# argmaxinc/WhisperKit

Hardware: AMD Instinct MI355X
Metric: audio-sec/sec (1/RTF), 30 s chunks: host PCM -> log-mel + encoder + greedy decode -> segments (higher is better)
Workload: dtype f16

## Files before the change

whisperkit_amd/csrc/epi_stage.h:

```cpp
#pragma once

#if defined(__HIPCC__)
#define WH_EPI_FN __host__ __device__ inline __attribute__((always_inline))
#else
#define WH_EPI_FN inline
#endif

namespace wh {
namespace epi {

constexpr int kWaveRegion = 16384;

constexpr int kRow16 = 144;
WH_EPI_FN int f16_write_off(int lane, int i2, int j, int g) { return (i2 * 32 + (lane & 31)) * kRow16 + j * 64 + g * 16 + (lane >> 5) * 8; }
WH_EPI_FN int f16_read_row(int lane, int it) { return it * 8 + (lane >> 3); }
WH_EPI_FN int f16_read_col(int lane) { return (lane & 7) * 8; }
WH_EPI_FN int f16_read_off(int lane, int it) { return f16_read_row(lane, it) * kRow16 + f16_read_col(lane) * 2; }

constexpr int kRow32 = 272;
WH_EPI_FN int f32_write_off(int lane, int j, int g) { return (lane & 31) * kRow32 + j * 128 + g * 32 + (lane >> 5) * 16; }
WH_EPI_FN int f32_read_row(int lane, int it) { return it * 4 + (lane >> 4); }
WH_EPI_FN int f32_read_col(int lane) { return (lane & 15) * 4; }
WH_EPI_FN int f32_read_off(int lane, int it) { return f32_read_row(lane, it) * kRow32 + f32_read_col(lane) * 4; }

constexpr int kRowT = 272;
WH_EPI_FN int vt_write_off(int lane, int i, int g) { return (lane & 31) * kRowT + (i * 32 + g * 8 + (lane >> 5) * 4) * 2; }
WH_EPI_FN int vt_read_col(int lane, int it) { return it * 4 + (lane >> 4); }
WH_EPI_FN int vt_read_row(int lane) { return (lane & 15) * 8; }
WH_EPI_FN int vt_read_off(int lane, int it) { return vt_read_col(lane, it) * kRowT + vt_read_row(lane) * 2; }

static_assert(64 * kRow16 <= kWaveRegion && 32 * kRow32 <= kWaveRegion && 32 * kRowT <= kWaveRegion, "a pass fits the wave's slice");

constexpr int kSplitStage = 3 * 16384;
WH_EPI_FN int split_swz(int row) { return (row >> 2) & 3; }
WH_EPI_FN int split_dma_row(int tid) { return tid >> 2; }
WH_EPI_FN int split_dma_chunk(int tid) { return (tid & 3) ^ split_swz(split_dma_row(tid)); }
WH_EPI_FN int split_read_off(int row, int chunk) { return row * 64 + ((chunk ^ split_swz(row)) * 16); }
static_assert(2 * kSplitStage <= 8 * kWaveRegion, "the split stages fit the launch's 128 KB (the staged epilogues' slices)");

}
}
```

whisperkit_amd/csrc/gemm.hip:

```cpp
#include <algorithm>
#include <cstdlib>
#include <type_traits>

#include "epi_stage.h"
#include "kernels.h"
#include "knobs.h"

namespace wh {

constexpr int BK = 32;
constexpr int LDT = 40;

template <int EPI, int TM, int TN, bool SPLIT = false>
__device__ __forceinline__ void gemm_epilogue(const GemmArgs& a, f32x16 (&acc)[TM][TN], int m_wave, int n_wave, int lane) {
#pragma unroll
    for (int j = 0; j < TN; ++j) {
        const int n = n_wave + j * 32 + (lane & 31);
        if (n >= a.N) continue;
        const float bias = a.bias ? a.bias[n] : 0.0f;
#pragma unroll
        for (int i = 0; i < TM; ++i) {
            const int mb = m_wave + i * 32 + 4 * (lane >> 5);
#pragma unroll
            for (int g = 0; g < 4; ++g) {
                const int mg = mb + 8 * g;
                if (mg >= a.M) continue;
                float v[4];
#pragma unroll
                for (int r = 0; r < 4; ++r) v[r] = acc[i][j][g * 4 + r] + bias;
                if constexpr (EPI == EPI_QKV_ENC) {
                    const int d = a.d_model;
                    if (n >= 2 * d) {
                        int call = n - 2 * d;
                        int bb = mg / kCtx, t = mg - bb * kCtx;
                        if (t + 3 < kCtx) {
                            f16x4 pk = {(f16)v[0], (f16)v[1], (f16)v[2], (f16)v[3]};
                            *reinterpret_cast<f16x4*>(a.vt16 + ((size_t)bb * d + call) * kCtxPad + t) = pk;
                        } else {
                            for (int r = 0; r < 4; ++r) {
                                int m = mg + r;
                                if (m < a.M) { int b2 = m / kCtx, t2 = m - b2 * kCtx; a.vt16[((size_t)b2 * d + call) * kCtxPad + t2] = (f16)v[r]; }
                            }
                        }
                        continue;
                    }
                }
#pragma unroll
                for (int r = 0; r < 4; ++r) {
                    const int m = mg + r;
                    if (m >= a.M) continue;
                    const float x = v[r];
                    if constexpr (EPI == EPI_F16) {
                        a.out16[(size_t)m * a.ldc + n] = (f16)x;
                    } else if constexpr (EPI == EPI_GELU_F16) {
                        if constexpr (SPLIT) { f16 h_, l_; split_f16(gelu_erf_fast(x), h_, l_); a.out16[(size_t)m * a.ldc + n] = h_; a.out16_lo[(size_t)m * a.ldc + n] = l_; }
                        else a.out16[(size_t)m * a.ldc + n] = (f16)gelu_erf_fast(x);
                    } else if constexpr (EPI == EPI_RESID_F32) {
                        a.out32[(size_t)m * a.ldc + n] += x;
                    } else if constexpr (EPI == EPI_F32) {
                        a.out32[(size_t)m * a.ldc + n] = x;
                    } else if constexpr (EPI == EPI_QKV_ENC) {
                        const int d = a.d_model;
                        if (n < d) a.out16[(size_t)m * d + n] = (f16)x;
                        else a.k16[(size_t)m * d + (n - d)] = (f16)x;
                    } else if constexpr (EPI == EPI_CROSS_KV) {
                        const int d = a.d_model, H = d >> 6;
                        const int l = n / (2 * d), rem = n - l * 2 * d, kv = rem >= d, hc = rem - kv * d;
                        const int bb = m / kCtx, t = m - bb * kCtx;
                        const size_t o = ((((size_t)l * a.max_batch + bb) * H + (hc >> 6)) * kCtx + t) * kHeadDim + (hc & 63);
                        f16 hi_; signed char lo_;
                        hr24_encode(x, hi_, lo_);
                        (kv ? a.kv_v_hi : a.kv_k_hi)[o] = hi_;
                        (kv ? a.kv_v_lo : a.kv_k_lo)[o] = lo_;
                    } else if constexpr (EPI == EPI_CONV1) {
                        int bb = m / a.rows_per_batch_out, t = m - bb * a.rows_per_batch_out;
                        if constexpr (SPLIT) {
                            const size_t o = ((size_t)bb * kFramesPad + t + 1) * a.ldc + n;
                            f16 h_, l_; split_f16(gelu_erf_fast(x), h_, l_); a.out16[o] = h_; a.out16_lo[o] = l_;
                        } else {
                            a.out16[((size_t)bb * kFramesPad + t + 1) * a.ldc + n] = (f16)gelu_erf_fast(x);
                        }
                    } else if constexpr (EPI == EPI_CONV2) {
                        int t = m % a.rows_per_batch_out;
                        a.out32[(size_t)m * a.ldc + n] = gelu_erf_fast(x) + a.pos[(size_t)t * a.ldc + n];
                    }
                }
            }
        }
    }
}

__device__ __forceinline__ void load_tile_bias(const GemmArgs& a, float4 (&bias)[2][4], int nw, int lane) {
#pragma unroll
    for (int j = 0; j < 2; ++j)
#pragma unroll
        for (int g = 0; g < 4; ++g) bias[j][g] = float4{0, 0, 0, 0};
    if (a.bias) {
#pragma unroll
        for (int j = 0; j < 2; ++j)
#pragma unroll
            for (int g = 0; g < 4; ++g) bias[j][g] = *reinterpret_cast<const float4*>(a.bias + nw + j * 32 + 8 * g + 4 * (lane >> 5));
    }
}

__device__ __forceinline__ void split_f16x4(float v0, float v1, float v2, float v3, f16x4& hi, f16x4& lo) {
    f16 h_, l_;
    split_f16(v0, h_, l_); hi[0] = h_; lo[0] = l_;
    split_f16(v1, h_, l_); hi[1] = h_; lo[1] = l_;
    split_f16(v2, h_, l_); hi[2] = h_; lo[2] = l_;
    split_f16(v3, h_, l_); hi[3] = h_; lo[3] = l_;
}

template <int EPI, int TM, int TN, bool BATCH_BIAS = false, bool SPLIT = false>
__device__ __forceinline__ void gemm_epilogue_swapped(const GemmArgs& a, f32x16 (&acc)[TM][TN], int m_wave, int n_wave, int lane) {
    float4 tile_bias[2][4];
    if constexpr (BATCH_BIAS) {
        static_assert(TM == 4 && TN == 2, "wave tile of gemm256_kernel");
        if (n_wave >= a.N) return;
        load_tile_bias(a, tile_bias, n_wave, lane);
    }
#pragma unroll
    for (int i = 0; i < TM; ++i) {
        const int m = m_wave + i * 32 + (lane & 31);
        if (m >= a.M) continue;
        int bb = 0, t = m;
        if constexpr (EPI == EPI_CROSS_KV) { bb = m / kCtx; t = m - bb * kCtx; }
        if constexpr (EPI == EPI_CONV1 || EPI == EPI_CONV2) { bb = m / a.rows_per_batch_out; t = m - bb * a.rows_per_batch_out; }
#pragma unroll
        for (int j = 0; j < TN; ++j) {
#pragma unroll
            for (int g = 0; g < 4; ++g) {
                const int n = n_wave + j * 32 + 8 * g + 4 * (lane >> 5);
                if (n >= a.N) continue;
                float4 bias = float4{0, 0, 0, 0};
                if constexpr (BATCH_BIAS) bias = tile_bias[j][g];
                else if (a.bias) bias = *reinterpret_cast<const float4*>(a.bias + n);
                float v0 = acc[i][j][4 * g] + bias.x, v1 = acc[i][j][4 * g + 1] + bias.y;
                float v2 = acc[i][j][4 * g + 2] + bias.z, v3 = acc[i][j][4 * g + 3] + bias.w;
                if constexpr (EPI == EPI_F16) {
                    *reinterpret_cast<f16x4*>(a.out16 + (size_t)m * a.ldc + n) = f16x4{(f16)v0, (f16)v1, (f16)v2, (f16)v3};
                } else if constexpr (EPI == EPI_GELU_F16) {
                    if constexpr (SPLIT) {
                        f16x4 hi, lo;
                        split_f16x4(gelu_erf_fast(v0), gelu_erf_fast(v1), gelu_erf_fast(v2), gelu_erf_fast(v3), hi, lo);
                        *reinterpret_cast<f16x4*>(a.out16 + (size_t)m * a.ldc + n) = hi;
                        *reinterpret_cast<f16x4*>(a.out16_lo + (size_t)m * a.ldc + n) = lo;
                    } else {
                        *reinterpret_cast<f16x4*>(a.out16 + (size_t)m * a.ldc + n) =
                            f16x4{(f16)gelu_erf_fast(v0), (f16)gelu_erf_fast(v1), (f16)gelu_erf_fast(v2), (f16)gelu_erf_fast(v3)};
                    }
                } else if constexpr (EPI == EPI_RESID_F32) {
                    float4* p = reinterpret_cast<float4*>(a.out32 + (size_t)m * a.ldc + n);
                    float4 o = *p;
                    o.x += v0; o.y += v1; o.z += v2; o.w += v3;
                    *p = o;
                } else if constexpr (EPI == EPI_F32) {
                    *reinterpret_cast<float4*>(a.out32 + (size_t)m * a.ldc + n) = float4{v0, v1, v2, v3};
                } else if constexpr (EPI == EPI_QKV_ENC) {
                    const int d = a.d_model;
                    f16* dst = n < d ? a.out16 + (size_t)m * d + n : a.k16 + (size_t)m * d + (n - d);
                    *reinterpret_cast<f16x4*>(dst) = f16x4{(f16)v0, (f16)v1, (f16)v2, (f16)v3};
                } else if constexpr (EPI == EPI_CROSS_KV) {
                    const int d = a.d_model, H = d >> 6;
                    const int l = n / (2 * d), rem = n - l * 2 * d, kv = rem >= d, hc = rem - kv * d;
                    const size_t o = ((((size_t)l * a.max_batch + bb) * H + (hc >> 6)) * kCtx + t) * kHeadDim + (hc & 63);
                    f16x4 hi4; char4 lo4;
                    { f16 h_; signed char l_; hr24_encode(v0, h_, l_); hi4[0] = h_; lo4.x = l_; hr24_encode(v1, h_, l_); hi4[1] = h_; lo4.y = l_;
                      hr24_encode(v2, h_, l_); hi4[2] = h_; lo4.z = l_; hr24_encode(v3, h_, l_); hi4[3] = h_; lo4.w = l_; }
                    *reinterpret_cast<f16x4*>((kv ? a.kv_v_hi : a.kv_k_hi) + o) = hi4;
                    *reinterpret_cast<char4*>((kv ? a.kv_v_lo : a.kv_k_lo) + o) = lo4;
                } else if constexpr (EPI == EPI_CONV1) {
                    if constexpr (SPLIT) {
                        const size_t o = ((size_t)bb * kFramesPad + t + 1) * a.ldc + n;
                        f16x4 hi, lo;
                        split_f16x4(gelu_erf_fast(v0), gelu_erf_fast(v1), gelu_erf_fast(v2), gelu_erf_fast(v3), hi, lo);
                        *reinterpret_cast<f16x4*>(a.out16 + o) = hi;
                        *reinterpret_cast<f16x4*>(a.out16_lo + o) = lo;
                    } else {
                        *reinterpret_cast<f16x4*>(a.out16 + ((size_t)bb * kFramesPad + t + 1) * a.ldc + n) =
                            f16x4{(f16)gelu_erf_fast(v0), (f16)gelu_erf_fast(v1), (f16)gelu_erf_fast(v2), (f16)gelu_erf_fast(v3)};
                    }
                } else if constexpr (EPI == EPI_CONV2) {
                    const float4 ps = *reinterpret_cast<const float4*>(a.pos + (size_t)t * a.ldc + n);
                    *reinterpret_cast<float4*>(a.out32 + (size_t)m * a.ldc + n) =
                        float4{gelu_erf_fast(v0) + ps.x, gelu_erf_fast(v1) + ps.y, gelu_erf_fast(v2) + ps.z, gelu_erf_fast(v3) + ps.w};
                }
            }
        }
    }
}

template <int BM, int BN, int EPI, bool SPLIT>
__device__ __forceinline__ void gemm_main(const GemmArgs& a) {
    constexpr int WM = BM / 2, WN = BN / 2, TM = WM / 32, TN = WN / 32;
    constexpr int CA = BM * 4 / 256, CB = BN * 4 / 256;
    __shared__ __attribute__((aligned(16))) f16 As[SPLIT ? 4 : 2][BM * LDT];
    __shared__ __attribute__((aligned(16))) f16 Bs[2][BN * LDT];

    const int tid = threadIdx.x, lane = tid & 63, wave = tid >> 6;
    const int wm = wave >> 1, wn = wave & 1;
    const int m0 = blockIdx.y * BM, n0 = blockIdx.x * BN;

    const f16* a_ptr[CA];
    const f16* a_lo_ptr[SPLIT ? CA : 1];
    bool a_ok[CA];
    int a_lds[CA];
#pragma unroll
    for (int i = 0; i < CA; ++i) {
        int c = tid + 256 * i, row = c >> 2, cc = c & 3;
        int m = m0 + row;
        a_ok[i] = m < a.M;
        int mm = a_ok[i] ? m : 0;
        long long off = (long long)(mm / a.a_rows_per_batch) * a.a_batch_stride + (long long)(mm % a.a_rows_per_batch) * a.lda;
        a_ptr[i] = a.A + off + cc * 8;
        if constexpr (SPLIT) a_lo_ptr[i] = a.A_lo + off + cc * 8;
        a_lds[i] = row * LDT + cc * 8;
    }
    const f16* b_ptr[CB];
    bool b_ok[CB];
    int b_lds[CB];
#pragma unroll
    for (int i = 0; i < CB; ++i) {
        int c = tid + 256 * i, row = c >> 2, cc = c & 3;
        int n = n0 + row;
        b_ok[i] = n < a.N;
        b_ptr[i] = a.W + (long long)(b_ok[i] ? n : 0) * a.K + cc * 8;
        b_lds[i] = row * LDT + cc * 8;
    }
    const int kc = (tid & 3) * 8;

    uint4 ra[CA], rb[CB], ral[SPLIT ? CA : 1];
    auto gload = [&](int k0) {
        bool kin = (k0 + kc) < a.K;
#pragma unroll
        for (int i = 0; i < CA; ++i) ra[i] = (a_ok[i] && kin) ? *reinterpret_cast<const uint4*>(a_ptr[i] + k0) : uint4{0, 0, 0, 0};
        if constexpr (SPLIT) {
#pragma unroll
            for (int i = 0; i < CA; ++i) ral[i] = (a_ok[i] && kin) ? *reinterpret_cast<const uint4*>(a_lo_ptr[i] + k0) : uint4{0, 0, 0, 0};
        }
#pragma unroll
        for (int i = 0; i < CB; ++i) rb[i] = (b_ok[i] && kin) ? *reinterpret_cast<const uint4*>(b_ptr[i] + k0) : uint4{0, 0, 0, 0};
    };
    auto lstore = [&](int buf) {
#pragma unroll
        for (int i = 0; i < CA; ++i) *reinterpret_cast<uint4*>(&As[buf][a_lds[i]]) = ra[i];
#pragma unroll
        for (int i = 0; i < CB; ++i) *reinterpret_cast<uint4*>(&Bs[buf][b_lds[i]]) = rb[i];
        if constexpr (SPLIT) {
#pragma unroll
            for (int i = 0; i < CA; ++i) *reinterpret_cast<uint4*>(&As[2 + buf][a_lds[i]]) = ral[i];
        }
    };

    const int nk = (a.K + BK - 1) / BK;
    const int fr = lane & 31, fk = (lane >> 5) * 8;
    auto body = [&](auto swap_tag) {
        constexpr bool SWAP = decltype(swap_tag)::value;
        f32x16 acc[TM][TN];
#pragma unroll
        for (int i = 0; i < TM; ++i)
#pragma unroll
            for (int j = 0; j < TN; ++j)
#pragma unroll
                for (int r = 0; r < 16; ++r) acc[i][j][r] = 0.0f;
        gload(0);
        lstore(0);
        __syncthreads();
        for (int kt = 0; kt < nk; ++kt) {
            const int cur = kt & 1;
            if (kt + 1 < nk) gload((kt + 1) * BK);
#pragma unroll
            for (int ks = 0; ks < 2; ++ks) {
                f16x8 af[TM], bf[TN];
#pragma unroll
                for (int i = 0; i < TM; ++i) af[i] = *reinterpret_cast<const f16x8*>(&As[cur][(wm * WM + i * 32 + fr) * LDT + ks * 16 + fk]);
#pragma unroll
                for (int j = 0; j < TN; ++j) bf[j] = *reinterpret_cast<const f16x8*>(&Bs[cur][(wn * WN + j * 32 + fr) * LDT + ks * 16 + fk]);
                f16x8 afl[SPLIT ? TM : 1];
                if constexpr (SPLIT) {
#pragma unroll
                    for (int i = 0; i < TM; ++i) afl[i] = *reinterpret_cast<const f16x8*>(&As[2 + cur][(wm * WM + i * 32 + fr) * LDT + ks * 16 + fk]);
                }
#pragma unroll
                for (int i = 0; i < TM; ++i)
#pragma unroll
                    for (int j = 0; j < TN; ++j) {
                        if constexpr (SWAP) acc[i][j] = __builtin_amdgcn_mfma_f32_32x32x16_f16(bf[j], af[i], acc[i][j], 0, 0, 0);
                        else acc[i][j] = __builtin_amdgcn_mfma_f32_32x32x16_f16(af[i], bf[j], acc[i][j], 0, 0, 0);
                        if constexpr (SPLIT) {
                            if constexpr (SWAP) acc[i][j] = __builtin_amdgcn_mfma_f32_32x32x16_f16(bf[j], afl[i], acc[i][j], 0, 0, 0);
                            else acc[i][j] = __builtin_amdgcn_mfma_f32_32x32x16_f16(afl[i], bf[j], acc[i][j], 0, 0, 0);
                        }
                    }
            }
            if (kt + 1 < nk) lstore(cur ^ 1);
            __syncthreads();
        }
        if constexpr (SWAP) gemm_epilogue_swapped<EPI, TM, TN, false, SPLIT>(a, acc, m0 + wm * WM, n0 + wn * WN, lane);
        else gemm_epilogue<EPI, TM, TN, SPLIT>(a, acc, m0 + wm * WM, n0 + wn * WN, lane);
    };
    if constexpr (EPI == EPI_QKV_ENC) {
        if (n0 + wn * WN >= 2 * a.d_model) body(std::false_type{});
        else body(std::true_type{});
    } else {
        body(std::true_type{});
    }
}

template <int BM, int BN, int EPI>
__global__ __launch_bounds__(256, 2) void gemm_kernel(const GemmArgs a) { gemm_main<BM, BN, EPI, false>(a); }
template <int BM, int BN, int EPI>
__global__ __launch_bounds__(256, 2) void gemm_split_kernel(const GemmArgs a) { gemm_main<BM, BN, EPI, true>(a); }

__device__ __forceinline__ void wave_lds_turn() {
    __builtin_amdgcn_fence(__ATOMIC_RELEASE, "wavefront");
    __builtin_amdgcn_wave_barrier();
    __builtin_amdgcn_fence(__ATOMIC_ACQUIRE, "wavefront");
}

template <int EPI, bool SPLIT = false>
__device__ __forceinline__ void epi_staged_f16(const GemmArgs& a, f32x16 (&acc)[4][2], unsigned char* wl, int mw, int nw, int lane) {
    if (nw >= a.N) return;
    f16* base = a.out16;
    int ld = a.ldc, nc = nw;
    if constexpr (EPI == EPI_QKV_ENC) {
        ld = a.d_model;
        if (nw >= ld) { base = a.k16; nc = nw - ld; }
    }
    float4 bias[2][4];
    load_tile_bias(a, bias, nw, lane);
    static_assert(!SPLIT || EPI == EPI_GELU_F16, "split output planes: GELU(fc1) only");
#pragma unroll
    for (int hh = 0; hh < 2; ++hh) {
#pragma unroll
        for (int plane = 0; plane < (SPLIT ? 2 : 1); ++plane) {
#pragma unroll
            for (int i2 = 0; i2 < 2; ++i2)
#pragma unroll
                for (int j = 0; j < 2; ++j)
#pragma unroll
                    for (int g = 0; g < 4; ++g) {
                        const f32x16& c = acc[2 * hh + i2][j];
                        const float v0 = c[4 * g] + bias[j][g].x, v1 = c[4 * g + 1] + bias[j][g].y, v2 = c[4 * g + 2] + bias[j][g].z, v3 = c[4 * g + 3] + bias[j][g].w;
                        f16x4 pk;
                        if constexpr (SPLIT) {
                            f16x4 hi, lo;
                            split_f16x4(gelu_erf_fast(v0), gelu_erf_fast(v1), gelu_erf_fast(v2), gelu_erf_fast(v3), hi, lo);
                            pk = plane ? lo : hi;
                        } else if constexpr (EPI == EPI_GELU_F16) pk = f16x4{(f16)gelu_erf_fast(v0), (f16)gelu_erf_fast(v1), (f16)gelu_erf_fast(v2), (f16)gelu_erf_fast(v3)};
                        else pk = f16x4{(f16)v0, (f16)v1, (f16)v2, (f16)v3};
                        *reinterpret_cast<f16x4*>(wl + epi::f16_write_off(lane, i2, j, g)) = pk;
                    }
            wave_lds_turn();
            f16* const dst = SPLIT && plane ? a.out16_lo : base;
#pragma unroll
            for (int it = 0; it < 8; ++it) {
                const int m = mw + hh * 64 + epi::f16_read_row(lane, it);
                const uint4 v = *reinterpret_cast<const uint4*>(wl + epi::f16_read_off(lane, it));
                if (m < a.M) *reinterpret_cast<uint4*>(dst + (size_t)m * ld + nc + epi::f16_read_col(lane)) = v;
            }
            wave_lds_turn();
        }
    }
}

__device__ __forceinline__ void epi_staged_resid(const GemmArgs& a, f32x16 (&acc)[4][2], unsigned char* wl, int mw, int nw, int lane) {
    if (nw >= a.N) return;
    float4 bias[2][4];
    load_tile_bias(a, bias, nw, lane);
#pragma unroll
    for (int i = 0; i < 4; ++i) {
        const int m_first = mw + i * 32 + epi::f32_read_row(lane, 0);
        float* const col0 = a.out32 + nw + epi::f32_read_col(lane);
        float4 old[8];
#pragma unroll
        for (int it = 0; it < 8; ++it) old[it] = *reinterpret_cast<const float4*>(col0 + (size_t)min(m_first + it * 4, a.M - 1) * a.ldc);
#pragma unroll
        for (int j = 0; j < 2; ++j)
#pragma unroll
            for (int g = 0; g < 4; ++g) {
                const f32x16& c = acc[i][j];
                *reinterpret_cast<float4*>(wl + epi::f32_write_off(lane, j, g)) =
                    float4{c[4 * g] + bias[j][g].x, c[4 * g + 1] + bias[j][g].y, c[4 * g + 2] + bias[j][g].z, c[4 * g + 3] + bias[j][g].w};
            }
        wave_lds_turn();
#pragma unroll
        for (int it = 0; it < 8; ++it) {
            const float4 v = *reinterpret_cast<const float4*>(wl + epi::f32_read_off(lane, it));
            float4 o = old[it];
            o.x += v.x; o.y += v.y; o.z += v.z; o.w += v.w;
            if (m_first + it * 4 < a.M) *reinterpret_cast<float4*>(col0 + (size_t)(m_first + it * 4) * a.ldc) = o;
        }
        wave_lds_turn();
    }
}

__device__ __forceinline__ void epi_staged_vt(const GemmArgs& a, f32x16 (&acc)[4][2], unsigned char* wl, int mw, int nw, int lane) {
    if (nw >= a.N) return;
    const int d = a.d_model;
    float bias2[2] = {0.0f, 0.0f};
    if (a.bias) { bias2[0] = a.bias[nw + (lane & 31)]; bias2[1] = a.bias[nw + 32 + (lane & 31)]; }
#pragma unroll
    for (int j = 0; j < 2; ++j) {
        const float bias = bias2[j];
#pragma unroll
        for (int i = 0; i < 4; ++i)
#pragma unroll
            for (int g = 0; g < 4; ++g) {
                const f32x16& c = acc[i][j];
                *reinterpret_cast<f16x4*>(wl + epi::vt_write_off(lane, i, g)) =
                    f16x4{(f16)(c[4 * g] + bias), (f16)(c[4 * g + 1] + bias), (f16)(c[4 * g + 2] + bias), (f16)(c[4 * g + 3] + bias)};
            }
        wave_lds_turn();
#pragma unroll
        for (int it = 0; it < 8; ++it) {
            const uint4 v = *reinterpret_cast<const uint4*>(wl + epi::vt_read_off(lane, it));
            const int call = nw - 2 * d + j * 32 + epi::vt_read_col(lane, it);
            const int m = mw + epi::vt_read_row(lane);
            if (m < a.M) {
                const int bb = m / kCtx, t = m - bb * kCtx;
                *reinterpret_cast<uint2*>(a.vt16 + ((size_t)bb * d + call) * kCtxPad + t) = uint2{v.x, v.y};
            }
            if (m + 4 < a.M) {
                const int bb = (m + 4) / kCtx, t = m + 4 - bb * kCtx;
                *reinterpret_cast<uint2*>(a.vt16 + ((size_t)bb * d + call) * kCtxPad + t) = uint2{v.z, v.w};
            }
        }
        wave_lds_turn();
    }
}

template <int EPI>
constexpr bool kHasStagedEpilogue = plan::has_staged_epilogue(EPI);

template <int EPI, int MODE, bool SPLIT>
__device__ __forceinline__ void gemm256_main(const GemmArgs& a) {
    constexpr int TM = 4, TN = 2;
    constexpr int STAGE = SPLIT ? epi::kSplitStage : 65536;
    constexpr int NP = SPLIT ? 6 : 8;
    extern __shared__ __attribute__((aligned(1024))) unsigned char smem[];
    const int tid = threadIdx.x, lane = tid & 63, wave = tid >> 6;
    const int wm = wave >> 2, wn = wave & 3;

    const int nwg = gridDim.x, orig = blockIdx.x;
    const int xcd = orig & 7, q = nwg >> 3, r = nwg & 7;
    const int wg = (xcd < r ? xcd * (q + 1) : r * (q + 1) + (xcd - r) * q) + (orig >> 3);
    const int tiles_n = (a.N + 255) >> 8, tiles_m = (a.M + 255) >> 8;
    constexpr int GM = 8;
    const int gsz = GM * tiles_n, grp = wg / gsz, first_m = grp * GM;
    const int gm = min(tiles_m - first_m, GM), in_g = wg - grp * gsz;
    const int m0 = (first_m + in_g % gm) << 8, n0 = (in_g / gm) << 8;

    const f16* src[NP];
    if constexpr (SPLIT) {
        const int srow = epi::split_dma_row(tid);
        const int chunk = epi::split_dma_chunk(tid);
#pragma unroll
        for (int j = 0; j < 2; ++j) {
            const int m = min(m0 + j * 128 + srow, a.M - 1);
            const long long off = (long long)(m / a.a_rows_per_batch) * a.a_batch_stride + (long long)(m % a.a_rows_per_batch) * a.lda + chunk * 8;
            src[j] = a.A + off;
            src[2 + j] = a.A_lo + off;
            const int n = min(n0 + j * 128 + srow, a.N - 1);
            src[4 + j] = a.W + (long long)n * a.K + chunk * 8;
        }
    } else {
        const int srow = tid >> 3;
        const int chunk = (tid & 7) ^ ((tid >> 4) & 7);
#pragma unroll
        for (int j = 0; j < 4; ++j) {
            const int m = min(m0 + j * 64 + srow, a.M - 1);
            src[j] = a.A + (long long)(m / a.a_rows_per_batch) * a.a_batch_stride + (long long)(m % a.a_rows_per_batch) * a.lda + chunk * 8;
            const int n = min(n0 + j * 64 + srow, a.N - 1);
            src[4 + j] = a.W + (long long)n * a.K + chunk * 8;
        }
    }
    auto piece = [&](int p, int kt) {
        if constexpr (SPLIT) {
            unsigned char* dst = smem + (kt & 1) * STAGE + wave * 1024 + (p >> 1) * 16384 + (p & 1) * 8192;
            __builtin_amdgcn_global_load_lds((const __attribute__((address_space(1))) void*)(src[p] + kt * 32),
                                             (__attribute__((address_space(3))) void*)dst, 16, 0, 0);
        } else {
            unsigned char* dst = smem + (kt & 1) * 65536 + wave * 1024 + (p >> 2) * 32768 + (p & 3) * 8192;
            __builtin_amdgcn_global_load_lds((const __attribute__((address_space(1))) void*)(src[p] + kt * 64),
                                             (__attribute__((address_space(3))) void*)dst, 16, 0, 0);
        }
    };

    const int fr = lane & 31, fh = lane >> 5, swz = SPLIT ? epi::split_swz(fr) : (fr >> 1) & 7;
    const int a_row_off = SPLIT ? (wm * 128 + fr) * 64 : (wm * 128 + fr) * 128, b_row_off = SPLIT ? 32768 + (wn * 64 + fr) * 64 : 32768 + (wn * 64 + fr) * 128;
    const int nk = SPLIT ? a.K >> 5 : a.K >> 6;
#define PP_BAR() do { __builtin_amdgcn_sched_barrier(0); asm volatile("s_barrier" ::: "memory"); __builtin_amdgcn_sched_barrier(0); } while (0)
#define PP_XBAR() do { __builtin_amdgcn_sched_barrier(0); asm volatile("s_waitcnt lgkmcnt(0)\n\ts_barrier" ::: "memory"); __builtin_amdgcn_sched_barrier(0); } while (0)
#define PP_VMWAIT() do { __builtin_amdgcn_sched_barrier(0); asm volatile("s_waitcnt vmcnt(0)" ::: "memory"); } while (0)
    auto body = [&](auto swap_tag) {
        constexpr bool SWAP = decltype(swap_tag)::value;
        f32x16 acc[TM][TN];
#pragma unroll
        for (int i = 0; i < TM; ++i)
#pragma unroll
            for (int j = 0; j < TN; ++j)
#pragma unroll
                for (int e = 0; e < 16; ++e) acc[i][j][e] = 0.0f;
        f16x8 af[2][TM], bf[2][TN];
        auto X = [&](int kt, int h) {
            if constexpr (SPLIT) {
                const unsigned char* sb = smem + (kt & 1) * STAGE;
                const int slot = ((2 * h + fh) ^ swz) * 16;
#pragma unroll
                for (int j = 0; j < TN; ++j) bf[0][j] = *reinterpret_cast<const f16x8*>(sb + b_row_off + j * 2048 + slot);
#pragma unroll
                for (int i = 0; i < TM; ++i) af[0][i] = *reinterpret_cast<const f16x8*>(sb + a_row_off + i * 2048 + slot);
#pragma unroll
                for (int i = 0; i < TM; ++i) af[1][i] = *reinterpret_cast<const f16x8*>(sb + 16384 + a_row_off + i * 2048 + slot);
            } else {
                const unsigned char* sb = smem + (kt & 1) * 65536;
#pragma unroll
                for (int s2 = 0; s2 < 2; ++s2) {
                    const int slot = ((2 * (2 * h + s2) + fh) ^ swz) * 16;
#pragma unroll
                    for (int j = 0; j < TN; ++j) bf[s2][j] = *reinterpret_cast<const f16x8*>(sb + b_row_off + j * 4096 + slot);
#pragma unroll
                    for (int i = 0; i < TM; ++i) af[s2][i] = *reinterpret_cast<const f16x8*>(sb + a_row_off + i * 4096 + slot);
                }
            }
        };
        auto Y = [&](auto dma_tag, int dma_kt) {
            constexpr bool DMA = decltype(dma_tag)::value;
            __builtin_amdgcn_s_setprio(1);
            if constexpr (SPLIT) {
#pragma unroll
                for (int i = 0; i < TM; ++i) {
#pragma unroll
                    for (int j = 0; j < TN; ++j) {
#pragma unroll
                        for (int pl = 0; pl < 2; ++pl) {
                            if constexpr (SWAP) acc[i][j] = __builtin_amdgcn_mfma_f32_32x32x16_f16(bf[0][j], af[pl][i], acc[i][j], 0, 0, 0);
                            else acc[i][j] = __builtin_amdgcn_mfma_f32_32x32x16_f16(af[pl][i], bf[0][j], acc[i][j], 0, 0, 0);
                        }
                    }
                    if constexpr (DMA) {
                        __builtin_amdgcn_sched_barrier(0);
                        if (i < 2) { piece(2 * i, dma_kt); piece(2 * i + 1, dma_kt); }
                        else piece(2 + i, dma_kt);
                        __builtin_amdgcn_sched_barrier(0);
                    }
                }
            } else {
#pragma unroll
                for (int s2 = 0; s2 < 2; ++s2)
#pragma unroll
                    for (int i = 0; i < TM; ++i) {
#pragma unroll
                        for (int j = 0; j < TN; ++j) {
                            if constexpr (SWAP) acc[i][j] = __builtin_amdgcn_mfma_f32_32x32x16_f16(bf[s2][j], af[s2][i], acc[i][j], 0, 0, 0);
                            else acc[i][j] = __builtin_amdgcn_mfma_f32_32x32x16_f16(af[s2][i], bf[s2][j], acc[i][j], 0, 0, 0);
                        }
                        if constexpr (DMA) { __builtin_amdgcn_sched_barrier(0); piece(s2 * 4 + i, dma_kt); __builtin_amdgcn_sched_barrier(0); }
                    }
            }
            __builtin_amdgcn_s_setprio(0);
        };
        constexpr std::true_type kDma{};
        constexpr std::false_type kNoDma{};
#pragma unroll
        for (int p = 0; p < NP; ++p) piece(p, 0);
        PP_VMWAIT();
        PP_BAR();
        if (wm == 0) {
            for (int t = 0; t + 1 < nk; ++t) {
                X(t, 0); PP_XBAR();
                Y(kDma, t + 1); PP_BAR();
                X(t, 1); PP_XBAR();
                Y(kNoDma, 0); PP_VMWAIT(); PP_BAR();
            }
            X(nk - 1, 0); PP_XBAR();
            Y(kNoDma, 0); PP_BAR();
            X(nk - 1, 1); PP_XBAR();
            Y(kNoDma, 0); PP_BAR();
            PP_BAR();
        } else {
            if (nk > 1) {
#pragma unroll
                for (int p = 0; p < NP; ++p) piece(p, 1);
            }
            PP_BAR();
            for (int t = 0; t + 2 < nk; ++t) {
                X(t, 0); PP_XBAR();
                Y(kNoDma, 0); PP_BAR();
                X(t, 1); PP_VMWAIT(); PP_XBAR();
                Y(kDma, t + 2); PP_BAR();
            }
            for (int t = max(nk - 2, 0); t < nk; ++t) {
                X(t, 0); PP_XBAR();
                Y(kNoDma, 0); PP_BAR();
                X(t, 1); PP_VMWAIT(); PP_XBAR();
                Y(kNoDma, 0); PP_BAR();
            }
        }
        if constexpr (MODE == 1 && kHasStagedEpilogue<EPI>) {
            unsigned char* wl = smem + wave * epi::kWaveRegion;
            if constexpr (!SWAP) epi_staged_vt(a, acc, wl, m0 + wm * 128, n0 + wn * 64, lane);
            else if constexpr (EPI == EPI_RESID_F32) epi_staged_resid(a, acc, wl, m0 + wm * 128, n0 + wn * 64, lane);
            else epi_staged_f16<EPI, SPLIT && EPI == EPI_GELU_F16>(a, acc, wl, m0 + wm * 128, n0 + wn * 64, lane);
        } else if constexpr (SWAP) gemm_epilogue_swapped<EPI, TM, TN, MODE == 2, SPLIT>(a, acc, m0 + wm * 128, n0 + wn * 64, lane);
        else gemm_epilogue<EPI, TM, TN, SPLIT>(a, acc, m0 + wm * 128, n0 + wn * 64, lane);
    };
#undef PP_BAR
#undef PP_XBAR
#undef PP_VMWAIT
    if constexpr (EPI == EPI_QKV_ENC) {
        if (n0 + wn * 64 >= 2 * a.d_model) body(std::false_type{});
        else body(std::true_type{});
    } else {
        body(std::true_type{});
    }
}

template <int EPI, int MODE>
__global__ __launch_bounds__(512) void gemm256_kernel(const GemmArgs a) { gemm256_main<EPI, MODE, false>(a); }
template <int EPI, int MODE>
__global__ __launch_bounds__(512) void gemm256_split_kernel(const GemmArgs a) { gemm256_main<EPI, MODE, true>(a); }


constexpr int kPersistWaveRegion = 12288;
static_assert(64 * epi::kRow16 <= kPersistWaveRegion && 32 * epi::kRow32 <= kPersistWaveRegion && 32 * epi::kRowT <= kPersistWaveRegion, "a pass fits the wave's slice");
template <int EPI, int MODE>
__global__ __launch_bounds__(512) void gemm256p_kernel(const GemmArgs a, int n_tiles, int stagger, int GM) {
    constexpr int TM = 4, TN = 2;
    extern __shared__ __attribute__((aligned(1024))) unsigned char smem[];
    const int tid = threadIdx.x, lane = tid & 63, wave = tid >> 6;
    const int wm = wave >> 2, wn = wave & 3;

    const int orig = blockIdx.x, xcd = orig & 7, q = n_tiles >> 3, r = n_tiles & 7;
    const int lo = xcd < r ? xcd * (q + 1) : r * (q + 1) + (xcd - r) * q, cnt = q + (xcd < r ? 1 : 0);
    const int per_xcd = gridDim.x >> 3;
    int it = orig >> 3;
    if (it >= cnt) return;
    if (stagger > 0) {
        const int rank = (it & 7) * 4 + ((it >> 3) & 3);
        for (int i = 0; i < rank * stagger; ++i) __builtin_amdgcn_s_sleep(1);
    }
    const int tiles_n = (a.N + 255) >> 8, tiles_m = (a.M + 255) >> 8;
    int m0, n0;
    auto tile_origin = [&](int wg, int& m0_, int& n0_) {
        const int gsz = GM * tiles_n, grp = wg / gsz, first_m = grp * GM;
        const int gm = min(tiles_m - first_m, GM), in_g = wg - grp * gsz;
        m0_ = (first_m + in_g % gm) << 8; n0_ = (in_g / gm) << 8;
    };
    const int srow = tid >> 3;
    const int chunk = (tid & 7) ^ ((tid >> 4) & 7);
    const f16* src[8];
    auto set_src = [&](int m0_, int n0_) {
#pragma unroll
        for (int j = 0; j < 4; ++j) {
            const int m = min(m0_ + j * 64 + srow, a.M - 1);
            src[j] = a.A + (long long)(m / a.a_rows_per_batch) * a.a_batch_stride + (long long)(m % a.a_rows_per_batch) * a.lda + chunk * 8;
            const int n = min(n0_ + j * 64 + srow, a.N - 1);
            src[4 + j] = a.W + (long long)n * a.K + chunk * 8;
        }
    };
    tile_origin(lo + it, m0, n0);
    set_src(m0, n0);
    auto piece = [&](int p, int kt) {
        unsigned char* dst = smem + (kt & 1) * 65536 + wave * 1024 + (p >> 2) * 32768 + (p & 3) * 8192;
        __builtin_amdgcn_global_load_lds((const __attribute__((address_space(1))) void*)(src[p] + kt * 64),
                                         (__attribute__((address_space(3))) void*)dst, 16, 0, 0);
    };

    const int fr = lane & 31, fh = lane >> 5, swz = (fr >> 1) & 7;
    const int a_row_off = (wm * 128 + fr) * 128, b_row_off = 32768 + (wn * 64 + fr) * 128;
    const int nk = a.K >> 6;
#define PP_BAR() do { __builtin_amdgcn_sched_barrier(0); asm volatile("s_barrier" ::: "memory"); __builtin_amdgcn_sched_barrier(0); } while (0)
#define PP_XBAR() do { __builtin_amdgcn_sched_barrier(0); asm volatile("s_waitcnt lgkmcnt(0)\n\ts_barrier" ::: "memory"); __builtin_amdgcn_sched_barrier(0); } while (0)
#define PP_VMWAIT() do { __builtin_amdgcn_sched_barrier(0); if (stagger != -2) asm volatile("s_waitcnt vmcnt(0)" ::: "memory"); } while (0)
    bool have_next = false;
    int m0n = 0, n0n = 0;
    auto body = [&](auto swap_tag) {
        constexpr bool SWAP = decltype(swap_tag)::value;
        f32x16 acc[TM][TN];
#pragma unroll
        for (int i = 0; i < TM; ++i)
#pragma unroll
            for (int j = 0; j < TN; ++j)
#pragma unroll
                for (int e = 0; e < 16; ++e) acc[i][j][e] = 0.0f;
        f16x8 af[2][TM], bf[2][TN];
        auto X = [&](int kt, int h) {
            const unsigned char* sb = smem + (kt & 1) * 65536;
#pragma unroll
            for (int s2 = 0; s2 < 2; ++s2) {
                const int slot = ((2 * (2 * h + s2) + fh) ^ swz) * 16;
#pragma unroll
                for (int j = 0; j < TN; ++j) bf[s2][j] = *reinterpret_cast<const f16x8*>(sb + b_row_off + j * 4096 + slot);
#pragma unroll
                for (int i = 0; i < TM; ++i) af[s2][i] = *reinterpret_cast<const f16x8*>(sb + a_row_off + i * 4096 + slot);
            }
        };
        auto Y = [&](auto dma_tag, int dma_kt) {
            constexpr bool DMA = decltype(dma_tag)::value;
            __builtin_amdgcn_s_setprio(1);
#pragma unroll
            for (int s2 = 0; s2 < 2; ++s2)
#pragma unroll
                for (int i = 0; i < TM; ++i) {
#pragma unroll
                    for (int j = 0; j < TN; ++j) {
                        if constexpr (SWAP) acc[i][j] = __builtin_amdgcn_mfma_f32_32x32x16_f16(bf[s2][j], af[s2][i], acc[i][j], 0, 0, 0);
                        else acc[i][j] = __builtin_amdgcn_mfma_f32_32x32x16_f16(af[s2][i], bf[s2][j], acc[i][j], 0, 0, 0);
                    }
                    if constexpr (DMA) { __builtin_amdgcn_sched_barrier(0); if (stagger != -1) piece(s2 * 4 + i, dma_kt); __builtin_amdgcn_sched_barrier(0); }
                }
            __builtin_amdgcn_s_setprio(0);
        };
        constexpr std::true_type kDma{};
        constexpr std::false_type kNoDma{};
        PP_VMWAIT();
        PP_BAR();
        if (wm == 0) {
            for (int t = 0; t + 1 < nk; ++t) {
                X(t, 0); PP_XBAR();
                Y(kDma, t + 1); PP_BAR();
                X(t, 1); PP_XBAR();
                Y(kNoDma, 0); PP_VMWAIT(); PP_BAR();
            }
            X(nk - 1, 0); PP_XBAR();
            Y(kNoDma, 0); PP_BAR();
            X(nk - 1, 1); PP_XBAR();
            Y(kNoDma, 0); PP_BAR();
            PP_BAR();
        } else {
            if (nk > 1) {
#pragma unroll
                for (int p = 0; p < 8; ++p) piece(p, 1);
            }
            PP_BAR();
            for (int t = 0; t + 2 < nk; ++t) {
                X(t, 0); PP_XBAR();
                Y(kNoDma, 0); PP_BAR();
                X(t, 1); PP_VMWAIT(); PP_XBAR();
                Y(kDma, t + 2); PP_BAR();
            }
            for (int t = max(nk - 2, 0); t < nk; ++t) {
                X(t, 0); PP_XBAR();
                Y(kNoDma, 0); PP_BAR();
                X(t, 1); PP_VMWAIT(); PP_XBAR();
                Y(kNoDma, 0); PP_BAR();
            }
        }
        const int m0c = m0, n0c = n0;
        {
            const int nx = it + per_xcd;
            have_next = nx < cnt;
            if (have_next) {
                tile_origin(lo + nx, m0n, n0n);
                set_src(m0n, n0n);
                __builtin_amdgcn_sched_barrier(0);
#pragma unroll
                for (int p = 0; p < 8; ++p) piece(p, 0);
                __builtin_amdgcn_sched_barrier(0);
            }
        }
        if constexpr (MODE == 1 && kHasStagedEpilogue<EPI>) {
            unsigned char* wl = smem + 65536 + wave * kPersistWaveRegion;
            if constexpr (!SWAP) epi_staged_vt(a, acc, wl, m0c + wm * 128, n0c + wn * 64, lane);
            else if constexpr (EPI == EPI_RESID_F32) epi_staged_resid(a, acc, wl, m0c + wm * 128, n0c + wn * 64, lane);
            else epi_staged_f16<EPI>(a, acc, wl, m0c + wm * 128, n0c + wn * 64, lane);
        } else if constexpr (SWAP) gemm_epilogue_swapped<EPI, TM, TN, MODE == 2>(a, acc, m0c + wm * 128, n0c + wn * 64, lane);
        else gemm_epilogue<EPI, TM, TN>(a, acc, m0c + wm * 128, n0c + wn * 64, lane);
    };
#undef PP_BAR
#undef PP_XBAR
#undef PP_VMWAIT
#pragma unroll
    for (int p = 0; p < 8; ++p) piece(p, 0);
    while (true) {
        if constexpr (EPI == EPI_QKV_ENC) {
            if (n0 + wn * 64 >= 2 * a.d_model) body(std::false_type{});
            else body(std::true_type{});
        } else {
            body(std::true_type{});
        }
        if (!have_next) break;
        it += per_xcd; m0 = m0n; n0 = n0n;
    }
}

static int persist_cus() {
    static PerDeviceOnce asked;
    static int cus = 256;
    asked.run([] { int dev = 0, n = 0; if (hipGetDevice(&dev) == hipSuccess && hipDeviceGetAttribute(&n, hipDeviceAttributeMultiprocessorCount, dev) == hipSuccess && n >= 8) cus = n / 8 * 8; });
    return cus;
}

template <int EPI, bool SPLIT>
static void launch_epi(const GemmArgs& a, hipStream_t st) {
    using namespace knob;
    uintptr_t bases = (uintptr_t)a.out16 | (uintptr_t)a.out32 | (uintptr_t)a.k16 | (uintptr_t)a.vt16;
    if constexpr (SPLIT) bases |= (uintptr_t)a.out16_lo;
    const int persist = SPLIT ? 0 : once<WH_GEMM_PERSIST>();
    const plan::GemmKnobs k{once<WH_NO_GEMM256>(), once<WH_GEMM_EPI_MODE>(), persist, persist ? once<WH_GEMM_PERSIST_WGS>() : 0, persist ? persist_cus() : 0};
    const plan::GemmPlan p = plan::gemm_plan(a.M, a.N, a.K, a.lda, a.a_batch_stride, a.ldc, a.d_model, EPI, SPLIT, bases, k);
    auto go256 = [&](auto mode_tag) {
        constexpr int MODE = decltype(mode_tag)::value;
        if constexpr (SPLIT) {
            static PerDeviceOnce raised;
            raised.run([] { (void)hipFuncSetAttribute(reinterpret_cast<const void*>(&gemm256_split_kernel<EPI, MODE>), hipFuncAttributeMaxDynamicSharedMemorySize, 131072); });
            gemm256_split_kernel<EPI, MODE><<<p.grid_x, 512, 131072, st>>>(a);
        } else if (p.family == plan::GEMM_256P) {
            static PerDeviceOnce raised_p;
            raised_p.run([] { (void)hipFuncSetAttribute(reinterpret_cast<const void*>(&gemm256p_kernel<EPI, MODE>), hipFuncAttributeMaxDynamicSharedMemorySize, 163840); });
            gemm256p_kernel<EPI, MODE><<<p.grid_x, 512, 163840, st>>>(a, (int)p.tiles256, once<WH_GEMM_STAGGER>(), once<WH_GEMM_GM>());
        } else {
            static PerDeviceOnce raised;
            raised.run([] { (void)hipFuncSetAttribute(reinterpret_cast<const void*>(&gemm256_kernel<EPI, MODE>), hipFuncAttributeMaxDynamicSharedMemorySize, 131072); });
            gemm256_kernel<EPI, MODE><<<p.grid_x, 512, 131072, st>>>(a);
        }
    };
    const dim3 g(p.grid_x, p.grid_y);
    switch (p.family) {
        case plan::GEMM_256:
        case plan::GEMM_256P:
            if constexpr (kHasStagedEpilogue<EPI>) {
                if (p.mode == 1) { go256(std::integral_constant<int, 1>{}); return; }
                if (p.mode == 2) { go256(std::integral_constant<int, 2>{}); return; }
            }
            go256(std::integral_constant<int, 0>{});
            return;
        case plan::GEMM_128:
            if constexpr (SPLIT) gemm_split_kernel<128, 128, EPI><<<g, 256, 0, st>>>(a); else gemm_kernel<128, 128, EPI><<<g, 256, 0, st>>>(a);
            return;
        case plan::GEMM_64:
            if constexpr (SPLIT) gemm_split_kernel<64, 64, EPI><<<g, 256, 0, st>>>(a); else gemm_kernel<64, 64, EPI><<<g, 256, 0, st>>>(a);
            return;
    }
}

void launch_gemm(GemmEpi epi, const GemmArgs& a, hipStream_t st) {
    ProfScope ps_(a.prof_kind, st);
#define GEMM_EPI_CASE(E_) case E_: if (a.A_lo) launch_epi<E_, true>(a, st); else launch_epi<E_, false>(a, st); break
    switch (epi) {
        GEMM_EPI_CASE(EPI_F16); GEMM_EPI_CASE(EPI_GELU_F16); GEMM_EPI_CASE(EPI_RESID_F32); GEMM_EPI_CASE(EPI_QKV_ENC);
        GEMM_EPI_CASE(EPI_CONV1); GEMM_EPI_CASE(EPI_CONV2); GEMM_EPI_CASE(EPI_F32); GEMM_EPI_CASE(EPI_CROSS_KV);
    }
#undef GEMM_EPI_CASE
}

}
```

Measured before the change: 2594.

## Switch non-split GEMM paths to 16x16x32 MFMA with swizzled LDS fragments

Introduces a WaveAcc abstraction that lets GEMM kernels use either 32x32x16 or 16x16x32 f16 MFMA tiles. The non-split GEMMs, including the persistent 256 kernel, move to the 16x16 instruction, with new swizzled LDS layouts and epilogue write offsets to match. The k-loop is factored into a shared gemm256_kloop. The aim is to cut LDS bank conflicts and improve MFMA issue density and latency. In exchange it issues more MFMA instructions per tile, changes how accumulator registers are laid out, and risks new scheduling or bank-conflict behaviour.

```diff
diff --git a/whisperkit_amd/csrc/epi_stage.h b/whisperkit_amd/csrc/epi_stage.h
--- a/whisperkit_amd/csrc/epi_stage.h
+++ b/whisperkit_amd/csrc/epi_stage.h
@@ -31,6 +31,20 @@
 
 static_assert(64 * kRow16 <= kWaveRegion && 32 * kRow32 <= kWaveRegion && 32 * kRowT <= kWaveRegion, "a pass fits the wave's slice");
 
+WH_EPI_FN int m16_own(int lane) { return lane & 15; }
+WH_EPI_FN int m16_quad(int lane) { return 4 * (lane >> 4); }
+WH_EPI_FN int f16_write_off_m16(int lane, int i4, int j) { return (i4 * 16 + m16_own(lane)) * kRow16 + (j * 16 + m16_quad(lane)) * 2; }
+WH_EPI_FN int f32_write_off_m16(int lane, int i2, int j) { return (i2 * 16 + m16_own(lane)) * kRow32 + (j * 16 + m16_quad(lane)) * 4; }
+WH_EPI_FN int vt_write_off_m16(int lane, int i, int j2) { return (j2 * 16 + m16_own(lane)) * kRowT + (i * 16 + m16_quad(lane)) * 2; }
+
+WH_EPI_FN int frag256_swz(int row) { return (row >> 1) & 7; }
+WH_EPI_FN int frag256_read_off(int row, int chunk) { return row * 128 + ((chunk ^ frag256_swz(row)) * 16); }
+WH_EPI_FN int m16_frag_row(int lane) { return lane & 15; }
+WH_EPI_FN int m16_frag_chunk(int lane, int h) { return 4 * h + (lane >> 4); }
+constexpr int kLdt16 = 32;
+WH_EPI_FN int frag64_swz(int row) { return (4 - ((row >> 2) & 3)) & 3; }
+WH_EPI_FN int frag64_off(int row, int chunk) { return row * kLdt16 + ((chunk ^ frag64_swz(row)) * 8); }
+
 constexpr int kSplitStage = 3 * 16384;
 WH_EPI_FN int split_swz(int row) { return (row >> 2) & 3; }
 WH_EPI_FN int split_dma_row(int tid) { return tid >> 2; }
diff --git a/whisperkit_amd/csrc/gemm.hip b/whisperkit_amd/csrc/gemm.hip
--- a/whisperkit_amd/csrc/gemm.hip
+++ b/whisperkit_amd/csrc/gemm.hip
@@ -11,23 +11,49 @@
 constexpr int BK = 32;
 constexpr int LDT = 40;
 
-template <int EPI, int TM, int TN, bool SPLIT = false>
-__device__ __forceinline__ void gemm_epilogue(const GemmArgs& a, f32x16 (&acc)[TM][TN], int m_wave, int n_wave, int lane) {
-#pragma unroll
-    for (int j = 0; j < TN; ++j) {
-        const int n = n_wave + j * 32 + (lane & 31);
+template <bool MF16, int TM, int TN>
+struct WaveAcc {
+    static constexpr bool kM16 = MF16;
+    static constexpr int R = MF16 ? 16 : 32, NI = TM * 32 / R, NJ = TN * 32 / R, NG = MF16 ? 1 : 4;
+    std::conditional_t<MF16, f32x4, f32x16> t[NI][NJ];
+    __device__ __forceinline__ void zero() {
+#pragma unroll
+        for (int i = 0; i < NI; ++i)
+#pragma unroll
+            for (int j = 0; j < NJ; ++j)
+#pragma unroll
+                for (int e = 0; e < 4 * NG; ++e) t[i][j][e] = 0.0f;
+    }
+    static __device__ __forceinline__ int own(int lane) { return MF16 ? epi::m16_own(lane) : lane & 31; }
+    static __device__ __forceinline__ int quad(int lane, int g) { return MF16 ? epi::m16_quad(lane) : 8 * g + 4 * (lane >> 5); }
+    template <bool SWAP>
+    __device__ __forceinline__ void mma(int i, int j, const f16x8& af, const f16x8& wf) {
+        if constexpr (MF16) {
+            if constexpr (SWAP) t[i][j] = __builtin_amdgcn_mfma_f32_16x16x32_f16(wf, af, t[i][j], 0, 0, 0);
+            else t[i][j] = __builtin_amdgcn_mfma_f32_16x16x32_f16(af, wf, t[i][j], 0, 0, 0);
+        } else {
+            if constexpr (SWAP) t[i][j] = __builtin_amdgcn_mfma_f32_32x32x16_f16(wf, af, t[i][j], 0, 0, 0);
+            else t[i][j] = __builtin_amdgcn_mfma_f32_32x32x16_f16(af, wf, t[i][j], 0, 0, 0);
+        }
+    }
+};
+
+template <int EPI, bool SPLIT = false, class ACC>
+__device__ __forceinline__ void gemm_epilogue(const GemmArgs& a, ACC& acc, int m_wave, int n_wave, int lane) {
+#pragma unroll
+    for (int j = 0; j < ACC::NJ; ++j) {
+        const int n = n_wave + j * ACC::R + ACC::own(lane);
         if (n >= a.N) continue;
         const float bias = a.bias ? a.bias[n] : 0.0f;
 #pragma unroll
-        for (int i = 0; i < TM; ++i) {
-            const int mb = m_wave + i * 32 + 4 * (lane >> 5);
-#pragma unroll
-            for (int g = 0; g < 4; ++g) {
-                const int mg = mb + 8 * g;
+        for (int i = 0; i < ACC::NI; ++i) {
+#pragma unroll
+            for (int g = 0; g < ACC::NG; ++g) {
+                const int mg = m_wave + i * ACC::R + ACC::quad(lane, g);
                 if (mg >= a.M) continue;
                 float v[4];
 #pragma unroll
-                for (int r = 0; r < 4; ++r) v[r] = acc[i][j][g * 4 + r] + bias;
+                for (int r = 0; r < 4; ++r) v[r] = acc.t[i][j][g * 4 + r] + bias;
                 if constexpr (EPI == EPI_QKV_ENC) {
                     const int d = a.d_model;
                     if (n >= 2 * d) {
@@ -90,16 +116,17 @@
     }
 }
 
-__device__ __forceinline__ void load_tile_bias(const GemmArgs& a, float4 (&bias)[2][4], int nw, int lane) {
-#pragma unroll
-    for (int j = 0; j < 2; ++j)
-#pragma unroll
-        for (int g = 0; g < 4; ++g) bias[j][g] = float4{0, 0, 0, 0};
+template <class ACC>
+__device__ __forceinline__ void load_tile_bias(const GemmArgs& a, float4 (&bias)[ACC::NJ][ACC::NG], int nw, int lane) {
+#pragma unroll
+    for (int j = 0; j < ACC::NJ; ++j)
+#pragma unroll
+        for (int g = 0; g < ACC::NG; ++g) bias[j][g] = float4{0, 0, 0, 0};
     if (a.bias) {
 #pragma unroll
-        for (int j = 0; j < 2; ++j)
-#pragma unroll
-            for (int g = 0; g < 4; ++g) bias[j][g] = *reinterpret_cast<const float4*>(a.bias + nw + j * 32 + 8 * g + 4 * (lane >> 5));
+        for (int j = 0; j < ACC::NJ; ++j)
+#pragma unroll
+            for (int g = 0; g < ACC::NG; ++g) bias[j][g] = *reinterpret_cast<const float4*>(a.bias + nw + j * ACC::R + ACC::quad(lane, g));
     }
 }
 
@@ -111,32 +138,32 @@
     split_f16(v3, h_, l_); hi[3] = h_; lo[3] = l_;
 }
 
-template <int EPI, int TM, int TN, bool BATCH_BIAS = false, bool SPLIT = false>
-__device__ __forceinline__ void gemm_epilogue_swapped(const GemmArgs& a, f32x16 (&acc)[TM][TN], int m_wave, int n_wave, int lane) {
-    float4 tile_bias[2][4];
+template <int EPI, bool BATCH_BIAS = false, bool SPLIT = false, class ACC>
+__device__ __forceinline__ void gemm_epilogue_swapped(const GemmArgs& a, ACC& acc, int m_wave, int n_wave, int lane) {
+    float4 tile_bias[ACC::NJ][ACC::NG];
     if constexpr (BATCH_BIAS) {
-        static_assert(TM == 4 && TN == 2, "wave tile of gemm256_kernel");
+        static_assert(ACC::NI * ACC::R == 128 && ACC::NJ * ACC::R == 64, "wave tile of gemm256_kernel");
         if (n_wave >= a.N) return;
-        load_tile_bias(a, tile_bias, n_wave, lane);
-    }
-#pragma unroll
-    for (int i = 0; i < TM; ++i) {
-        const int m = m_wave + i * 32 + (lane & 31);
+        load_tile_bias<ACC>(a, tile_bias, n_wave, lane);
+    }
+#pragma unroll
+    for (int i = 0; i < ACC::NI; ++i) {
+        const int m = m_wave + i * ACC::R + ACC::own(lane);
         if (m >= a.M) continue;
         int bb = 0, t = m;
         if constexpr (EPI == EPI_CROSS_KV) { bb = m / kCtx; t = m - bb * kCtx; }
         if constexpr (EPI == EPI_CONV1 || EPI == EPI_CONV2) { bb = m / a.rows_per_batch_out; t = m - bb * a.rows_per_batch_out; }
 #pragma unroll
-        for (int j = 0; j < TN; ++j) {
-#pragma unroll
-            for (int g = 0; g < 4; ++g) {
-                const int n = n_wave + j * 32 + 8 * g + 4 * (lane >> 5);
+        for (int j = 0; j < ACC::NJ; ++j) {
+#pragma unroll
+            for (int g = 0; g < ACC::NG; ++g) {
+                const int n = n_wave + j * ACC::R + ACC::quad(lane, g);
                 if (n >= a.N) continue;
                 float4 bias = float4{0, 0, 0, 0};
                 if constexpr (BATCH_BIAS) bias = tile_bias[j][g];
                 else if (a.bias) bias = *reinterpret_cast<const float4*>(a.bias + n);
-                float v0 = acc[i][j][4 * g] + bias.x, v1 = acc[i][j][4 * g + 1] + bias.y;
-                float v2 = acc[i][j][4 * g + 2] + bias.z, v3 = acc[i][j][4 * g + 3] + bias.w;
+                float v0 = acc.t[i][j][4 * g] + bias.x, v1 = acc.t[i][j][4 * g + 1] + bias.y;
+                float v2 = acc.t[i][j][4 * g + 2] + bias.z, v3 = acc.t[i][j][4 * g + 3] + bias.w;
                 if constexpr (EPI == EPI_F16) {
                     *reinterpret_cast<f16x4*>(a.out16 + (size_t)m * a.ldc + n) = f16x4{(f16)v0, (f16)v1, (f16)v2, (f16)v3};
                 } else if constexpr (EPI == EPI_GELU_F16) {
@@ -192,10 +219,13 @@
 
 template <int BM, int BN, int EPI, bool SPLIT>
 __device__ __forceinline__ void gemm_main(const GemmArgs& a) {
-    constexpr int WM = BM / 2, WN = BN / 2, TM = WM / 32, TN = WN / 32;
+    constexpr bool MF16 = !SPLIT;
+    using Acc = WaveAcc<MF16, BM / 64, BN / 64>;
+    constexpr int WM = BM / 2, WN = BN / 2, R = Acc::R;
     constexpr int CA = BM * 4 / 256, CB = BN * 4 / 256;
-    __shared__ __attribute__((aligned(16))) f16 As[SPLIT ? 4 : 2][BM * LDT];
-    __shared__ __attribute__((aligned(16))) f16 Bs[2][BN * LDT];
+    constexpr int LDR = MF16 ? epi::kLdt16 : LDT;
+    __shared__ __attribute__((aligned(256))) f16 As[SPLIT ? 4 : 2][BM * LDR];
+    __shared__ __attribute__((aligned(256))) f16 Bs[2][BN * LDR];
 
     const int tid = threadIdx.x, lane = tid & 63, wave = tid >> 6;
     const int wm = wave >> 1, wn = wave & 1;
@@ -214,7 +244,7 @@
         long long off = (long long)(mm / a.a_rows_per_batch) * a.a_batch_stride + (long long)(mm % a.a_rows_per_batch) * a.lda;
         a_ptr[i] = a.A + off + cc * 8;
         if constexpr (SPLIT) a_lo_ptr[i] = a.A_lo + off + cc * 8;
-        a_lds[i] = row * LDT + cc * 8;
+        a_lds[i] = MF16 ? epi::frag64_off(row, cc) : row * LDT + cc * 8;
     }
     const f16* b_ptr[CB];
     bool b_ok[CB];
@@ -225,7 +255,7 @@
         int n = n0 + row;
         b_ok[i] = n < a.N;
         b_ptr[i] = a.W + (long long)(b_ok[i] ? n : 0) * a.K + cc * 8;
-        b_lds[i] = row * LDT + cc * 8;
+        b_lds[i] = MF16 ? epi::frag64_off(row, cc) : row * LDT + cc * 8;
     }
     const int kc = (tid & 3) * 8;
 
@@ -253,16 +283,12 @@
     };
 
     const int nk = (a.K + BK - 1) / BK;
-    const int fr = lane & 31, fk = (lane >> 5) * 8;
+    const int fr = lane & (R - 1), fk = (lane >> 5) * 8;
     auto body = [&](auto swap_tag) {
         constexpr bool SWAP = decltype(swap_tag)::value;
-        f32x16 acc[TM][TN];
-#pragma unroll
-        for (int i = 0; i < TM; ++i)
-#pragma unroll
-            for (int j = 0; j < TN; ++j)
-#pragma unroll
-                for (int r = 0; r < 16; ++r) acc[i][j][r] = 0.0f;
+        constexpr int TM = Acc::NI, TN = Acc::NJ;
+        Acc acc;
+        acc.zero();
         gload(0);
         lstore(0);
         __syncthreads();
@@ -270,34 +296,31 @@
             const int cur = kt & 1;
             if (kt + 1 < nk) gload((kt + 1) * BK);
 #pragma unroll
-            for (int ks = 0; ks < 2; ++ks) {
+            for (int ks = 0; ks < (MF16 ? 1 : 2); ++ks) {
                 f16x8 af[TM], bf[TN];
-#pragma unroll
-                for (int i = 0; i < TM; ++i) af[i] = *reinterpret_cast<const f16x8*>(&As[cur][(wm * WM + i * 32 + fr) * LDT + ks * 16 + fk]);
-#pragma unroll
-                for (int j = 0; j < TN; ++j) bf[j] = *reinterpret_cast<const f16x8*>(&Bs[cur][(wn * WN + j * 32 + fr) * LDT + ks * 16 + fk]);
+                auto frag = [&](int row) { return MF16 ? epi::frag64_off(row, lane >> 4) : row * LDT + ks * 16 + fk; };
+#pragma unroll
+                for (int i = 0; i < TM; ++i) af[i] = *reinterpret_cast<const f16x8*>(&As[cur][frag(wm * WM + i * R + fr)]);
+#pragma unroll
+                for (int j = 0; j < TN; ++j) bf[j] = *reinterpret_cast<const f16x8*>(&Bs[cur][frag(wn * WN + j * R + fr)]);
                 f16x8 afl[SPLIT ? TM : 1];
                 if constexpr (SPLIT) {
 #pragma unroll
-                    for (int i = 0; i < TM; ++i) afl[i] = *reinterpret_cast<const f16x8*>(&As[2 + cur][(wm * WM + i * 32 + fr) * LDT + ks * 16 + fk]);
+                    for (int i = 0; i < TM; ++i) afl[i] = *reinterpret_cast<const f16x8*>(&As[2 + cur][frag(wm * WM + i * R + fr)]);
                 }
 #pragma unroll
                 for (int i = 0; i < TM; ++i)
 #pragma unroll
                     for (int j = 0; j < TN; ++j) {
-                        if constexpr (SWAP) acc[i][j] = __builtin_amdgcn_mfma_f32_32x32x16_f16(bf[j], af[i], acc[i][j], 0, 0, 0);
-                        else acc[i][j] = __builtin_amdgcn_mfma_f32_32x32x16_f16(af[i], bf[j], acc[i][j], 0, 0, 0);
-                        if constexpr (SPLIT) {
-                            if constexpr (SWAP) acc[i][j] = __builtin_amdgcn_mfma_f32_32x32x16_f16(bf[j], afl[i], acc[i][j], 0, 0, 0);
-                            else acc[i][j] = __builtin_amdgcn_mfma_f32_32x32x16_f16(afl[i], bf[j], acc[i][j], 0, 0, 0);
-                        }
+                        acc.template mma<SWAP>(i, j, af[i], bf[j]);
+                        if constexpr (SPLIT) acc.template mma<SWAP>(i, j, afl[i], bf[j]);
                     }
             }
             if (kt + 1 < nk) lstore(cur ^ 1);
             __syncthreads();
         }
-        if constexpr (SWAP) gemm_epilogue_swapped<EPI, TM, TN, false, SPLIT>(a, acc, m0 + wm * WM, n0 + wn * WN, lane);
-        else gemm_epilogue<EPI, TM, TN, SPLIT>(a, acc, m0 + wm * WM, n0 + wn * WN, lane);
+        if constexpr (SWAP) gemm_epilogue_swapped<EPI, false, SPLIT>(a, acc, m0 + wm * WM, n0 + wn * WN, lane);
+        else gemm_epilogue<EPI, SPLIT>(a, acc, m0 + wm * WM, n0 + wn * WN, lane);
     };
     if constexpr (EPI == EPI_QKV_ENC) {
         if (n0 + wn * WN >= 2 * a.d_model) body(std::false_type{});
@@ -318,8 +341,9 @@
     __builtin_amdgcn_fence(__ATOMIC_ACQUIRE, "wavefront");
 }
 
-template <int EPI, bool SPLIT = false>
-__device__ __forceinline__ void epi_staged_f16(const GemmArgs& a, f32x16 (&acc)[4][2], unsigned char* wl, int mw, int nw, int lane) {
+template <int EPI, bool SPLIT = false, class ACC>
+__device__ __forceinline__ void epi_staged_f16(const GemmArgs& a, ACC& acc, unsigned char* wl, int mw, int nw, int lane) {
+    constexpr int IP = 64 / ACC::R;
     if (nw >= a.N) return;
     f16* base = a.out16;
     int ld = a.ldc, nc = nw;
@@ -327,20 +351,20 @@
         ld = a.d_model;
         if (nw >= ld) { base = a.k16; nc = nw - ld; }
     }
-    float4 bias[2][4];
-    load_tile_bias(a, bias, nw, lane);
+    float4 bias[ACC::NJ][ACC::NG];
+    load_tile_bias<ACC>(a, bias, nw, lane);
     static_assert(!SPLIT || EPI == EPI_GELU_F16, "split output planes: GELU(fc1) only");
 #pragma unroll
     for (int hh = 0; hh < 2; ++hh) {
 #pragma unroll
         for (int plane = 0; plane < (SPLIT ? 2 : 1); ++plane) {
 #pragma unroll
-            for (int i2 = 0; i2 < 2; ++i2)
-#pragma unroll
-                for (int j = 0; j < 2; ++j)
-#pragma unroll
-                    for (int g = 0; g < 4; ++g) {
-                        const f32x16& c = acc[2 * hh + i2][j];
+            for (int i2 = 0; i2 < IP; ++i2)
+#pragma unroll
+                for (int j = 0; j < ACC::NJ; ++j)
+#pragma unroll
+                    for (int g = 0; g < ACC::NG; ++g) {
+                        const auto& c = acc.t[IP * hh + i2][j];
                         const float v0 = c[4 * g] + bias[j][g].x, v1 = c[4 * g + 1] + bias[j][g].y, v2 = c[4 * g + 2] + bias[j][g].z, v3 = c[4 * g + 3] + bias[j][g].w;
                         f16x4 pk;
                         if constexpr (SPLIT) {
@@ -349,7 +373,7 @@
                             pk = plane ? lo : hi;
                         } else if constexpr (EPI == EPI_GELU_F16) pk = f16x4{(f16)gelu_erf_fast(v0), (f16)gelu_erf_fast(v1), (f16)gelu_erf_fast(v2), (f16)gelu_erf_fast(v3)};
                         else pk = f16x4{(f16)v0, (f16)v1, (f16)v2, (f16)v3};
-                        *reinterpret_cast<f16x4*>(wl + epi::f16_write_off(lane, i2, j, g)) = pk;
+                        *reinterpret_cast<f16x4*>(wl + (ACC::kM16 ? epi::f16_write_off_m16(lane, i2, j) : epi::f16_write_off(lane, i2, j, g))) = pk;
                     }
             wave_lds_turn();
             f16* const dst = SPLIT && plane ? a.out16_lo : base;
@@ -364,10 +388,12 @@
     }
 }
 
-__device__ __forceinline__ void epi_staged_resid(const GemmArgs& a, f32x16 (&acc)[4][2], unsigned char* wl, int mw, int nw, int lane) {
+template <class ACC>
+__device__ __forceinline__ void epi_staged_resid(const GemmArgs& a, ACC& acc, unsigned char* wl, int mw, int nw, int lane) {
+    constexpr int IP = 32 / ACC::R;
     if (nw >= a.N) return;
-    float4 bias[2][4];
-    load_tile_bias(a, bias, nw, lane);
+    float4 bias[ACC::NJ][ACC::NG];
+    load_tile_bias<ACC>(a, bias, nw, lane);
 #pragma unroll
     for (int i = 0; i < 4; ++i) {
         const int m_first = mw + i * 32 + epi::f32_read_row(lane, 0);
@@ -376,13 +402,15 @@
 #pragma unroll
         for (int it = 0; it < 8; ++it) old[it] = *reinterpret_cast<const float4*>(col0 + (size_t)min(m_first + it * 4, a.M - 1) * a.ldc);
 #pragma unroll
-        for (int j = 0; j < 2; ++j)
-#pragma unroll
-            for (int g = 0; g < 4; ++g) {
-                const f32x16& c = acc[i][j];
-                *reinterpret_cast<float4*>(wl + epi::f32_write_off(lane, j, g)) =
-                    float4{c[4 * g] + bias[j][g].x, c[4 * g + 1] + bias[j][g].y, c[4 * g + 2] + bias[j][g].z, c[4 * g + 3] + bias[j][g].w};
-            }
+        for (int i2 = 0; i2 < IP; ++i2)
+#pragma unroll
+            for (int j = 0; j < ACC::NJ; ++j)
+#pragma unroll
+                for (int g = 0; g < ACC::NG; ++g) {
+                    const auto& c = acc.t[IP * i + i2][j];
+                    *reinterpret_cast<float4*>(wl + (ACC::kM16 ? epi::f32_write_off_m16(lane, i2, j) : epi::f32_write_off(lane, j, g))) =
+                        float4{c[4 * g] + bias[j][g].x, c[4 * g + 1] + bias[j][g].y, c[4 * g + 2] + bias[j][g].z, c[4 * g + 3] + bias[j][g].w};
+                }
         wave_lds_turn();
 #pragma unroll
         for (int it = 0; it < 8; ++it) {
@@ -395,22 +423,32 @@
     }
 }
 
-__device__ __forceinline__ void epi_staged_vt(const GemmArgs& a, f32x16 (&acc)[4][2], unsigned char* wl, int mw, int nw, int lane) {
+template <class ACC>
+__device__ __forceinline__ void epi_staged_vt(const GemmArgs& a, ACC& acc, unsigned char* wl, int mw, int nw, int lane) {
+    constexpr int JP = 32 / ACC::R;
     if (nw >= a.N) return;
     const int d = a.d_model;
-    float bias2[2] = {0.0f, 0.0f};
-    if (a.bias) { bias2[0] = a.bias[nw + (lane & 31)]; bias2[1] = a.bias[nw + 32 + (lane & 31)]; }
+    float bias_j[ACC::NJ];
+#pragma unroll
+    for (int j = 0; j < ACC::NJ; ++j) bias_j[j] = 0.0f;
+    if (a.bias) {
+#pragma unroll
+        for (int j = 0; j < ACC::NJ; ++j) bias_j[j] = a.bias[nw + j * ACC::R + ACC::own(lane)];
+    }
 #pragma unroll
     for (int j = 0; j < 2; ++j) {
-        const float bias = bias2[j];
-#pragma unroll
-        for (int i = 0; i < 4; ++i)
-#pragma unroll
-            for (int g = 0; g < 4; ++g) {
-                const f32x16& c = acc[i][j];
-                *reinterpret_cast<f16x4*>(wl + epi::vt_write_off(lane, i, g)) =
-                    f16x4{(f16)(c[4 * g] + bias), (f16)(c[4 * g + 1] + bias), (f16)(c[4 * g + 2] + bias), (f16)(c[4 * g + 3] + bias)};
-            }
+#pragma unroll
+        for (int j2 = 0; j2 < JP; ++j2) {
+            const float bias = bias_j[JP * j + j2];
+#pragma unroll
+            for (int i = 0; i < ACC::NI; ++i)
+#pragma unroll
+                for (int g = 0; g < ACC::NG; ++g) {
+                    const auto& c = acc.t[i][JP * j + j2];
+                    *reinterpret_cast<f16x4*>(wl + (ACC::kM16 ? epi::vt_write_off_m16(lane, i, j2) : epi::vt_write_off(lane, i, g))) =
+                        f16x4{(f16)(c[4 * g] + bias), (f16)(c[4 * g + 1] + bias), (f16)(c[4 * g + 2] + bias), (f16)(c[4 * g + 3] + bias)};
+                }
+        }
         wave_lds_turn();
 #pragma unroll
         for (int it = 0; it < 8; ++it) {
@@ -433,9 +471,132 @@
 template <int EPI>
 constexpr bool kHasStagedEpilogue = plan::has_staged_epilogue(EPI);
 
-template <int EPI, int MODE, bool SPLIT>
+template <bool SWAP, bool SPLIT, bool FIRST, class ACC, class Piece>
+__device__ __forceinline__ void gemm256_kloop(ACC& acc, const unsigned char* smem, Piece piece, int nk, int wm, int wn, int lane, int probe) {
+    constexpr bool MF16 = ACC::kM16;
+    static_assert(!(SPLIT && MF16), "the split form keeps 32x32x16");
+    constexpr int TM = 4, TN = 2;
+    constexpr int STAGE = SPLIT ? epi::kSplitStage : 65536;
+    constexpr int NP = SPLIT ? 6 : 8;
+    const int fr = lane & (ACC::R - 1), fh = lane / ACC::R, swz = SPLIT ? epi::split_swz(fr) : epi::frag256_swz(fr);
+    const int a_row_off = SPLIT ? (wm * 128 + fr) * 64 : (wm * 128 + fr) * 128, b_row_off = SPLIT ? 32768 + (wn * 64 + fr) * 64 : 32768 + (wn * 64 + fr) * 128;
+#define PP_BAR() do { __builtin_amdgcn_sched_barrier(0); asm volatile("s_barrier" ::: "memory"); __builtin_amdgcn_sched_barrier(0); } while (0)
+#define PP_XBAR() do { __builtin_amdgcn_sched_barrier(0); asm volatile("s_waitcnt lgkmcnt(0)\n\ts_barrier" ::: "memory"); __builtin_amdgcn_sched_barrier(0); } while (0)
+#define PP_VMWAIT() do { __builtin_amdgcn_sched_barrier(0); if (probe != -2) asm volatile("s_waitcnt vmcnt(0)" ::: "memory"); } while (0)
+    f16x8 af[2 * TM], bf[2 * TN];
+    auto X = [&](int kt, int h) {
+        const unsigned char* sb = smem + (kt & 1) * STAGE;
+        if constexpr (SPLIT) {
+            const int slot = ((2 * h + fh) ^ swz) * 16;
+#pragma unroll
+            for (int j = 0; j < TN; ++j) bf[j] = *reinterpret_cast<const f16x8*>(sb + b_row_off + j * 2048 + slot);
+#pragma unroll
+            for (int i = 0; i < TM; ++i) af[i] = *reinterpret_cast<const f16x8*>(sb + a_row_off + i * 2048 + slot);
+#pragma unroll
+            for (int i = 0; i < TM; ++i) af[TM + i] = *reinterpret_cast<const f16x8*>(sb + 16384 + a_row_off + i * 2048 + slot);
+        } else if constexpr (MF16) {
+            const int slot = (epi::m16_frag_chunk(lane, h) ^ swz) * 16;
+#pragma unroll
+            for (int j = 0; j < ACC::NJ; ++j) bf[j] = *reinterpret_cast<const f16x8*>(sb + b_row_off + j * 2048 + slot);
+#pragma unroll
+            for (int i = 0; i < ACC::NI; ++i) af[i] = *reinterpret_cast<const f16x8*>(sb + a_row_off + i * 2048 + slot);
+        } else {
+#pragma unroll
+            for (int s2 = 0; s2 < 2; ++s2) {
+                const int slot = ((2 * (2 * h + s2) + fh) ^ swz) * 16;
+#pragma unroll
+                for (int j = 0; j < TN; ++j) bf[s2 * TN + j] = *reinterpret_cast<const f16x8*>(sb + b_row_off + j * 4096 + slot);
+#pragma unroll
+                for (int i = 0; i < TM; ++i) af[s2 * TM + i] = *reinterpret_cast<const f16x8*>(sb + a_row_off + i * 4096 + slot);
+            }
+        }
+    };
+    auto Y = [&](auto dma_tag, int dma_kt) {
+        constexpr bool DMA = decltype(dma_tag)::value;
+        __builtin_amdgcn_s_setprio(1);
+        if constexpr (SPLIT) {
+#pragma unroll
+            for (int i = 0; i < TM; ++i) {
+#pragma unroll
+                for (int j = 0; j < TN; ++j) {
+#pragma unroll
+                    for (int pl = 0; pl < 2; ++pl) acc.template mma<SWAP>(i, j, af[pl * TM + i], bf[j]);
+                }
+                if constexpr (DMA) {
+                    __builtin_amdgcn_sched_barrier(0);
+                    if (probe != -1) {
+                        if (i < 2) { piece(2 * i, dma_kt); piece(2 * i + 1, dma_kt); }
+                        else piece(2 + i, dma_kt);
+                    }
+                    __builtin_amdgcn_sched_barrier(0);
+                }
+            }
+        } else if constexpr (MF16) {
+#pragma unroll
+            for (int i = 0; i < ACC::NI; ++i) {
+#pragma unroll
+                for (int j = 0; j < ACC::NJ; ++j) acc.template mma<SWAP>(i, j, af[i], bf[j]);
+                if constexpr (DMA) { __builtin_amdgcn_sched_barrier(0); if (probe != -1) piece(i, dma_kt); __builtin_amdgcn_sched_barrier(0); }
+            }
+        } else {
+#pragma unroll
+            for (int s2 = 0; s2 < 2; ++s2)
+#pragma unroll
+                for (int i = 0; i < TM; ++i) {
+#pragma unroll
+                    for (int j = 0; j < TN; ++j) acc.template mma<SWAP>(i, j, af[s2 * TM + i], bf[s2 * TN + j]);
+                    if constexpr (DMA) { __builtin_amdgcn_sched_barrier(0); if (probe != -1) piece(s2 * 4 + i, dma_kt); __builtin_amdgcn_sched_barrier(0); }
+                }
+        }
+        __builtin_amdgcn_s_setprio(0);
+    };
+    constexpr std::true_type kDma{};
+    constexpr std::false_type kNoDma{};
+    if constexpr (FIRST) {
+#pragma unroll
+        for (int p = 0; p < NP; ++p) piece(p, 0);
+    }
+    PP_VMWAIT();
+    PP_BAR();
+    if (wm == 0) {
+        for (int t = 0; t + 1 < nk; ++t) {
+            X(t, 0); PP_XBAR();
+            Y(kDma, t + 1); PP_BAR();
+            X(t, 1); PP_XBAR();
+            Y(kNoDma, 0); PP_VMWAIT(); PP_BAR();
+        }
+        X(nk - 1, 0); PP_XBAR();
+        Y(kNoDma, 0); PP_BAR();
+        X(nk - 1, 1); PP_XBAR();
+        Y(kNoDma, 0); PP_BAR();
+        PP_BAR();
+    } else {
+        if (nk > 1) {
+#pragma unroll
+            for (int p = 0; p < NP; ++p) piece(p, 1);
+        }
+        PP_BAR();
+        for (int t = 0; t + 2 < nk; ++t) {
+            X(t, 0); PP_XBAR();
+            Y(kNoDma, 0); PP_BAR();
+            X(t, 1); PP_VMWAIT(); PP_XBAR();
+            Y(kDma, t + 2); PP_BAR();
+        }
+        for (int t = max(nk - 2, 0); t < nk; ++t) {
+            X(t, 0); PP_XBAR();
+            Y(kNoDma, 0); PP_BAR();
+            X(t, 1); PP_VMWAIT(); PP_XBAR();
+            Y(kNoDma, 0); PP_BAR();
+        }
+    }
+#undef PP_BAR
+#undef PP_XBAR
+#undef PP_VMWAIT
+}
+
+template <int EPI, int MODE, bool SPLIT, bool MF16 = !SPLIT>
 __device__ __forceinline__ void gemm256_main(const GemmArgs& a) {
-    constexpr int TM = 4, TN = 2;
+    using Acc = WaveAcc<MF16, 4, 2>;
     constexpr int STAGE = SPLIT ? epi::kSplitStage : 65536;
     constexpr int NP = SPLIT ? 6 : 8;
     extern __shared__ __attribute__((aligned(1024))) unsigned char smem[];
@@ -466,7 +627,7 @@
         }
     } else {
         const int srow = tid >> 3;
-        const int chunk = (tid & 7) ^ ((tid >> 4) & 7);
+        const int chunk = (tid & 7) ^ epi::frag256_swz(srow);
 #pragma unroll
         for (int j = 0; j < 4; ++j) {
             const int m = min(m0 + j * 64 + srow, a.M - 1);
@@ -486,129 +647,20 @@
                                              (__attribute__((address_space(3))) void*)dst, 16, 0, 0);
         }
     };
-
-    const int fr = lane & 31, fh = lane >> 5, swz = SPLIT ? epi::split_swz(fr) : (fr >> 1) & 7;
-    const int a_row_off = SPLIT ? (wm * 128 + fr) * 64 : (wm * 128 + fr) * 128, b_row_off = SPLIT ? 32768 + (wn * 64 + fr) * 64 : 32768 + (wn * 64 + fr) * 128;
     const int nk = SPLIT ? a.K >> 5 : a.K >> 6;
-#define PP_BAR() do { __builtin_amdgcn_sched_barrier(0); asm volatile("s_barrier" ::: "memory"); __builtin_amdgcn_sched_barrier(0); } while (0)
-#define PP_XBAR() do { __builtin_amdgcn_sched_barrier(0); asm volatile("s_waitcnt lgkmcnt(0)\n\ts_barrier" ::: "memory"); __builtin_amdgcn_sched_barrier(0); } while (0)
-#define PP_VMWAIT() do { __builtin_amdgcn_sched_barrier(0); asm volatile("s_waitcnt vmcnt(0)" ::: "memory"); } while (0)
     auto body = [&](auto swap_tag) {
         constexpr bool SWAP = decltype(swap_tag)::value;
-        f32x16 acc[TM][TN];
-#pragma unroll
-        for (int i = 0; i < TM; ++i)
-#pragma unroll
-            for (int j = 0; j < TN; ++j)
-#pragma unroll
-                for (int e = 0; e < 16; ++e) acc[i][j][e] = 0.0f;
-        f16x8 af[2][TM], bf[2][TN];
-        auto X = [&](int kt, int h) {
-            if constexpr (SPLIT) {
-                const unsigned char* sb = smem + (kt & 1) * STAGE;
-                const int slot = ((2 * h + fh) ^ swz) * 16;
-#pragma unroll
-                for (int j = 0; j < TN; ++j) bf[0][j] = *reinterpret_cast<const f16x8*>(sb + b_row_off + j * 2048 + slot);
-#pragma unroll
-                for (int i = 0; i < TM; ++i) af[0][i] = *reinterpret_cast<const f16x8*>(sb + a_row_off + i * 2048 + slot);
-#pragma unroll
-                for (int i = 0; i < TM; ++i) af[1][i] = *reinterpret_cast<const f16x8*>(sb + 16384 + a_row_off + i * 2048 + slot);
-            } else {
-                const unsigned char* sb = smem + (kt & 1) * 65536;
-#pragma unroll
-                for (int s2 = 0; s2 < 2; ++s2) {
-                    const int slot = ((2 * (2 * h + s2) + fh) ^ swz) * 16;
-#pragma unroll
-                    for (int j = 0; j < TN; ++j) bf[s2][j] = *reinterpret_cast<const f16x8*>(sb + b_row_off + j * 4096 + slot);
-#pragma unroll
-                    for (int i = 0; i < TM; ++i) af[s2][i] = *reinterpret_cast<const f16x8*>(sb + a_row_off + i * 4096 + slot);
-                }
-            }
-        };
-        auto Y = [&](auto dma_tag, int dma_kt) {
-            constexpr bool DMA = decltype(dma_tag)::value;
-            __builtin_amdgcn_s_setprio(1);
-            if constexpr (SPLIT) {
-#pragma unroll
-                for (int i = 0; i < TM; ++i) {
-#pragma unroll
-                    for (int j = 0; j < TN; ++j) {
-#pragma unroll
-                        for (int pl = 0; pl < 2; ++pl) {
-                            if constexpr (SWAP) acc[i][j] = __builtin_amdgcn_mfma_f32_32x32x16_f16(bf[0][j], af[pl][i], acc[i][j], 0, 0, 0);
-                            else acc[i][j] = __builtin_amdgcn_mfma_f32_32x32x16_f16(af[pl][i], bf[0][j], acc[i][j], 0, 0, 0);
-                        }
-                    }
-                    if constexpr (DMA) {
-                        __builtin_amdgcn_sched_barrier(0);
-                        if (i < 2) { piece(2 * i, dma_kt); piece(2 * i + 1, dma_kt); }
-                        else piece(2 + i, dma_kt);
-                        __builtin_amdgcn_sched_barrier(0);
-                    }
-                }
-            } else {
-#pragma unroll
-                for (int s2 = 0; s2 < 2; ++s2)
-#pragma unroll
-                    for (int i = 0; i < TM; ++i) {
-#pragma unroll
-                        for (int j = 0; j < TN; ++j) {
-                            if constexpr (SWAP) acc[i][j] = __builtin_amdgcn_mfma_f32_32x32x16_f16(bf[s2][j], af[s2][i], acc[i][j], 0, 0, 0);
-                            else acc[i][j] = __builtin_amdgcn_mfma_f32_32x32x16_f16(af[s2][i], bf[s2][j], acc[i][j], 0, 0, 0);
-                        }
-                        if constexpr (DMA) { __builtin_amdgcn_sched_barrier(0); piece(s2 * 4 + i, dma_kt); __builtin_amdgcn_sched_barrier(0); }
-                    }
-            }
-            __builtin_amdgcn_s_setprio(0);
-        };
-        constexpr std::true_type kDma{};
-        constexpr std::false_type kNoDma{};
-#pragma unroll
-        for (int p = 0; p < NP; ++p) piece(p, 0);
-        PP_VMWAIT();
-        PP_BAR();
-        if (wm == 0) {
-            for (int t = 0; t + 1 < nk; ++t) {
-                X(t, 0); PP_XBAR();
-                Y(kDma, t + 1); PP_BAR();
-                X(t, 1); PP_XBAR();
-                Y(kNoDma, 0); PP_VMWAIT(); PP_BAR();
-            }
-            X(nk - 1, 0); PP_XBAR();
-            Y(kNoDma, 0); PP_BAR();
-            X(nk - 1, 1); PP_XBAR();
-            Y(kNoDma, 0); PP_BAR();
-            PP_BAR();
-        } else {
-            if (nk > 1) {
-#pragma unroll
-                for (int p = 0; p < NP; ++p) piece(p, 1);
-            }
-            PP_BAR();
-            for (int t = 0; t + 2 < nk; ++t) {
-                X(t, 0); PP_XBAR();
-                Y(kNoDma, 0); PP_BAR();
-                X(t, 1); PP_VMWAIT(); PP_XBAR();
-                Y(kDma, t + 2); PP_BAR();
-            }
-            for (int t = max(nk - 2, 0); t < nk; ++t) {
-                X(t, 0); PP_XBAR();
-                Y(kNoDma, 0); PP_BAR();
-                X(t, 1); PP_VMWAIT(); PP_XBAR();
-                Y(kNoDma, 0); PP_BAR();
-            }
-        }
+        Acc acc;
+        acc.zero();
+        gemm256_kloop<SWAP, SPLIT, true>(acc, smem, piece, nk, wm, wn, lane, 0);
         if constexpr (MODE == 1 && kHasStagedEpilogue<EPI>) {
             unsigned char* wl = smem + wave * epi::kWaveRegion;
             if constexpr (!SWAP) epi_staged_vt(a, acc, wl, m0 + wm * 128, n0 + wn * 64, lane);
             else if constexpr (EPI == EPI_RESID_F32) epi_staged_resid(a, acc, wl, m0 + wm * 128, n0 + wn * 64, lane);
             else epi_staged_f16<EPI, SPLIT && EPI == EPI_GELU_F16>(a, acc, wl, m0 + wm * 128, n0 + wn * 64, lane);
-        } else if constexpr (SWAP) gemm_epilogue_swapped<EPI, TM, TN, MODE == 2, SPLIT>(a, acc, m0 + wm * 128, n0 + wn * 64, lane);
-        else gemm_epilogue<EPI, TM, TN, SPLIT>(a, acc, m0 + wm * 128, n0 + wn * 64, lane);
-    };
-#undef PP_BAR
-#undef PP_XBAR
-#undef PP_VMWAIT
+        } else if constexpr (SWAP) gemm_epilogue_swapped<EPI, MODE == 2, SPLIT>(a, acc, m0 + wm * 128, n0 + wn * 64, lane);
+        else gemm_epilogue<EPI, SPLIT>(a, acc, m0 + wm * 128, n0 + wn * 64, lane);
+    };
     if constexpr (EPI == EPI_QKV_ENC) {
         if (n0 + wn * 64 >= 2 * a.d_model) body(std::false_type{});
         else body(std::true_type{});
@@ -627,7 +679,6 @@
 static_assert(64 * epi::kRow16 <= kPersistWaveRegion && 32 * epi::kRow32 <= kPersistWaveRegion && 32 * epi::kRowT <= kPersistWaveRegion, "a pass fits the wave's slice");
 template <int EPI, int MODE>
 __global__ __launch_bounds__(512) void gemm256p_kernel(const GemmArgs a, int n_tiles, int stagger, int GM) {
-    constexpr int TM = 4, TN = 2;
     extern __shared__ __attribute__((aligned(1024))) unsigned char smem[];
     const int tid = threadIdx.x, lane = tid & 63, wave = tid >> 6;
     const int wm = wave >> 2, wn = wave & 3;
@@ -649,7 +700,7 @@
         m0_ = (first_m + in_g % gm) << 8; n0_ = (in_g / gm) << 8;
     };
     const int srow = tid >> 3;
-    const int chunk = (tid & 7) ^ ((tid >> 4) & 7);
+    const int chunk = (tid & 7) ^ epi::frag256_swz(srow);
     const f16* src[8];
     auto set_src = [&](int m0_, int n0_) {
 #pragma unroll
@@ -668,86 +719,14 @@
                                          (__attribute__((address_space(3))) void*)dst, 16, 0, 0);
     };
 
-    const int fr = lane & 31, fh = lane >> 5, swz = (fr >> 1) & 7;
-    const int a_row_off = (wm * 128 + fr) * 128, b_row_off = 32768 + (wn * 64 + fr) * 128;
     const int nk = a.K >> 6;
-#define PP_BAR() do { __builtin_amdgcn_sched_barrier(0); asm volatile("s_barrier" ::: "memory"); __builtin_amdgcn_sched_barrier(0); } while (0)
-#define PP_XBAR() do { __builtin_amdgcn_sched_barrier(0); asm volatile("s_waitcnt lgkmcnt(0)\n\ts_barrier" ::: "memory"); __builtin_amdgcn_sched_barrier(0); } while (0)
-#define PP_VMWAIT() do { __builtin_amdgcn_sched_barrier(0); if (stagger != -2) asm volatile("s_waitcnt vmcnt(0)" ::: "memory"); } while (0)
     bool have_next = false;
     int m0n = 0, n0n = 0;
     auto body = [&](auto swap_tag) {
         constexpr bool SWAP = decltype(swap_tag)::value;
-        f32x16 acc[TM][TN];
-#pragma unroll
-        for (int i = 0; i < TM; ++i)
-#pragma unroll
-            for (int j = 0; j < TN; ++j)
-#pragma unroll
-                for (int e = 0; e < 16; ++e) acc[i][j][e] = 0.0f;
-        f16x8 af[2][TM], bf[2][TN];
-        auto X = [&](int kt, int h) {
-            const unsigned char* sb = smem + (kt & 1) * 65536;
-#pragma unroll
-            for (int s2 = 0; s2 < 2; ++s2) {
-                const int slot = ((2 * (2 * h + s2) + fh) ^ swz) * 16;
-#pragma unroll
-                for (int j = 0; j < TN; ++j) bf[s2][j] = *reinterpret_cast<const f16x8*>(sb + b_row_off + j * 4096 + slot);
-#pragma unroll
-                for (int i = 0; i < TM; ++i) af[s2][i] = *reinterpret_cast<const f16x8*>(sb + a_row_off + i * 4096 + slot);
-            }
-        };
-        auto Y = [&](auto dma_tag, int dma_kt) {
-            constexpr bool DMA = decltype(dma_tag)::value;
-            __builtin_amdgcn_s_setprio(1);
-#pragma unroll
-            for (int s2 = 0; s2 < 2; ++s2)
-#pragma unroll
-                for (int i = 0; i < TM; ++i) {
-#pragma unroll
-                    for (int j = 0; j < TN; ++j) {
-                        if constexpr (SWAP) acc[i][j] = __builtin_amdgcn_mfma_f32_32x32x16_f16(bf[s2][j], af[s2][i], acc[i][j], 0, 0, 0);
-                        else acc[i][j] = __builtin_amdgcn_mfma_f32_32x32x16_f16(af[s2][i], bf[s2][j], acc[i][j], 0, 0, 0);
-                    }
-                    if constexpr (DMA) { __builtin_amdgcn_sched_barrier(0); if (stagger != -1) piece(s2 * 4 + i, dma_kt); __builtin_amdgcn_sched_barrier(0); }
-                }
-            __builtin_amdgcn_s_setprio(0);
-        };
-        constexpr std::true_type kDma{};
-        constexpr std::false_type kNoDma{};
-        PP_VMWAIT();
-        PP_BAR();
-        if (wm == 0) {
-            for (int t = 0; t + 1 < nk; ++t) {
-                X(t, 0); PP_XBAR();
-                Y(kDma, t + 1); PP_BAR();
-                X(t, 1); PP_XBAR();
-                Y(kNoDma, 0); PP_VMWAIT(); PP_BAR();
-            }
-            X(nk - 1, 0); PP_XBAR();
-            Y(kNoDma, 0); PP_BAR();
-            X(nk - 1, 1); PP_XBAR();
-            Y(kNoDma, 0); PP_BAR();
-            PP_BAR();
-        } else {
-            if (nk > 1) {
-#pragma unroll
-                for (int p = 0; p < 8; ++p) piece(p, 1);
-            }
-            PP_BAR();
-            for (int t = 0; t + 2 < nk; ++t) {
-                X(t, 0); PP_XBAR();
-                Y(kNoDma, 0); PP_BAR();
-                X(t, 1); PP_VMWAIT(); PP_XBAR();
-                Y(kDma, t + 2); PP_BAR();
-            }
-            for (int t = max(nk - 2, 0); t < nk; ++t) {
-                X(t, 0); PP_XBAR();
-                Y(kNoDma, 0); PP_BAR();
-                X(t, 1); PP_VMWAIT(); PP_XBAR();
-                Y(kNoDma, 0); PP_BAR();
-            }
-        }
+        WaveAcc<true, 4, 2> acc;
+        acc.zero();
+        gemm256_kloop<SWAP, false, false>(acc, smem, piece, nk, wm, wn, lane, stagger);
         const int m0c = m0, n0c = n0;
         {
             const int nx = it + per_xcd;
@@ -766,12 +745,9 @@
             if constexpr (!SWAP) epi_staged_vt(a, acc, wl, m0c + wm * 128, n0c + wn * 64, lane);
             else if constexpr (EPI == EPI_RESID_F32) epi_staged_resid(a, acc, wl, m0c + wm * 128, n0c + wn * 64, lane);
             else epi_staged_f16<EPI>(a, acc, wl, m0c + wm * 128, n0c + wn * 64, lane);
-        } else if constexpr (SWAP) gemm_epilogue_swapped<EPI, TM, TN, MODE == 2>(a, acc, m0c + wm * 128, n0c + wn * 64, lane);
-        else gemm_epilogue<EPI, TM, TN>(a, acc, m0c + wm * 128, n0c + wn * 64, lane);
-    };
-#undef PP_BAR
-#undef PP_XBAR
-#undef PP_VMWAIT
+        } else if constexpr (SWAP) gemm_epilogue_swapped<EPI, MODE == 2>(a, acc, m0c + wm * 128, n0c + wn * 64, lane);
+        else gemm_epilogue<EPI>(a, acc, m0c + wm * 128, n0c + wn * 64, lane);
+    };
 #pragma unroll
     for (int p = 0; p < 8; ++p) piece(p, 0);
     while (true) {
```

Result: no change. 2613 (median of 6 runs) (+0.8%).
